# stefanopini/simple-HRNet

Hardware: AMD Instinct MI355X
Metric: person-crops/sec HRNet-W48 384x288 (model forward + heat-map decode) (higher is better)
Workload: dtype bf16; 1 GPU; HRNet-W48 384x288, batch=256 random crops per GPU, bf16 MFMA (BASELINE configs[2]); global_batch=256, micro_batch=256, lanes_per_gpu=1, parallelism=dp1 (crop sharding, RCCL all-gather of keypoints), weights=random-init seeded (synth_state_dict seed 0), BN stats randomised, engine_switches=

## Files before the change

### include/hrnet_mi355.h

```cpp
#ifndef HRNET_MI355_H
#define HRNET_MI355_H

#include <stddef.h>
#include <stdint.h>

#ifdef __cplusplus
extern "C" {
#endif

typedef struct hrn_ctx *hrn_handle;

enum { HRN_F32 = 0, HRN_BF16 = 1, HRN_F16 = 2 };
enum { HRN_BOX_I32 = 0, HRN_BOX_F32 = 1 };
enum { HRN_T_F32 = 0, HRN_T_I64 = 1 };

typedef struct {
    const char *name;
    const void *data;
    int32_t ndim;
    int64_t dims[4];
    int32_t dtype;
} hrn_tensor_desc;

typedef struct {
// ... 70 lines not shown
int hrn_preprocess_frames_yuv_dev(hrn_handle h, const hrn_yuv_frame *frames_host, int nframes, const float *dets_dev,
                                  int det_stride, const int32_t *frame_index_host, int n, int variant, float *images_dev,
                                  int32_t *boxes_dev, int32_t *status_dev, void *stream);

#define HRN_MAX_TRACKED 256
int hrn_associate_people(int P, const int32_t *cur_start, const int32_t *prev_start, int J, int32_t *boxes, float *pts,
                         const int32_t *prev_boxes, const float *prev_pts, const int32_t *prev_ids, int32_t *next_id, double pose_alpha,
                         double similarity_threshold, double smoothing_alpha, int32_t *ids, int32_t *match, int32_t *status);
const char *hrn_associate_people_last_error(void);
int hrn_associate_people_dev(hrn_handle h, int P, const int32_t *cur_start_host, const int32_t *prev_start_host, int J,
                             int32_t *boxes_dev, float *pts_dev, const int32_t *prev_boxes_dev, const float *prev_pts_dev,
                             const int32_t *prev_ids_dev, int32_t *next_id_dev, double pose_alpha, double similarity_threshold,
                             double smoothing_alpha, int32_t *ids_dev, int32_t *match_dev, int32_t *status_dev, void *stream);
int hrn_assoc_exp(const double *x, int n, double *out);
int hrn_associate_similarity(const int32_t *boxes, const float *pts, int n, const int32_t *prev_boxes, const float *prev_pts, int m, int J,
                             double pose_alpha, double *cost_out , float *sim_out );

#define HRN_POSE_NMS_SOFT 1
#define HRN_POSE_NMS_SUPPRESS 2
#define HRN_POSE_NMS_ENGINE 4
int hrn_pose_nms(int P, const int32_t *start, int J, int flags, void *kpts, void *areas, const void *scores, double thresh,
                 double in_vis_thre, double rescore_thre, const double *sigmas, int32_t *keep, int32_t *num, double *scores_out,
                 int32_t *suppressor, int32_t *status);
const char *hrn_pose_nms_last_error(void);
int hrn_pose_nms_dev(hrn_handle h, int P, const int32_t *start_host, int J, int flags, void *kpts_dev, void *areas_dev,
                     const void *scores_dev, double thresh, double in_vis_thre, double rescore_thre, const double *sigmas_dev,
                     int32_t *keep_dev, int32_t *num_dev, double *scores_out_dev, int32_t *suppressor_dev, int32_t *status_dev,
                     void *stream);
int hrn_pose_nms_oks_row(int n, int J, int flags, const void *kpts, const void *areas, int g, double in_vis_thre, const double *sigmas,
                         double *oks_out );

enum { HRN_PIX_BGR = 0 };
typedef struct { uint8_t *y, *u, *v;
                 int32_t height, width, pitch_y, pitch_c, format, matrix, range; } hrn_canvas;
int hrn_draw_poses(hrn_handle h, const hrn_canvas *canvases_host, int nframes, const float *pts_dev, int n, int J,
                   const int32_t *frame_index_host , const int32_t *skeleton_host, int K,
                   const uint8_t *point_colors_host, int Cp, const uint8_t *bone_colors_host, int Cb,
                   const int32_t *person_index_host , int radius ,
                   int thickness, float threshold, void *stream);
int hrn_draw_poses_ids_dev(hrn_handle h, const hrn_canvas *canvases_host, int nframes, const float *pts_dev, int n, int J,
                           const int32_t *frame_index_host, const int32_t *skeleton_host, int K, const uint8_t *point_colors_host,
                           int Cp, const uint8_t *bone_colors_host, int Cb, const int32_t *person_index_dev, int radius,
                           int thickness, float threshold, void *stream);
int hrn_yuv_from_bgr(int matrix, int range, const uint8_t *bgr , int n, uint8_t *yuv_out );

enum { HRN_LETTERBOX_MAX_SIDE = 0, HRN_LETTERBOX_MIN_RATIO = 1 };
enum { HRN_LB_F32 = 0, HRN_LB_F16 = 1, HRN_LB_BF16 = 2, HRN_LB_U8_HWC = 3 };
enum { HRN_LB_RGB = 0, HRN_LB_BGR = 1 };
enum { HRN_DET_COMPACT = 1 };
enum { HRN_DET_MAX_CLASSES = 16 };
typedef struct { int32_t new_w, new_h, left, top; double ratio_w, ratio_h, dw, dh; } hrn_letterbox;
int hrn_letterbox_geometry(int rule, const int32_t *frame_hw , int n, int out_h, int out_w,
                           hrn_letterbox *out );
const char *hrn_letterbox_last_error(void);
int hrn_letterbox_frames(hrn_handle h, const hrn_frame *frames_host, int n, int rule, int out_h, int out_w,
                         const uint8_t *pad , int order, int form, void *out_dev, hrn_letterbox *geometry_host ,
                         void *stream);
int hrn_letterbox_frames_yuv(hrn_handle h, const hrn_yuv_frame *frames_host, int n, int rule, int out_h, int out_w,
                             const uint8_t *pad , int order, int form, void *out_dev,
                             hrn_letterbox *geometry_host , void *stream);
int hrn_detections_to_frame(int rule, const float *dets, int det_stride, const int32_t *start , int P,
                            const hrn_letterbox *geometry, const int32_t *frame_hw , int out_h, int out_w,
                            int conf_col, float conf_thres, int class_col, const int32_t *classes, int nclasses, int flags,
                            float *dets_out, int32_t *counts_out , int32_t *status_out );
int hrn_detections_to_frame_dev(hrn_handle h, int rule, const float *dets_dev, int det_stride, const int32_t *start_host, int P,
                                const hrn_letterbox *geometry_host, const int32_t *frame_hw_host, int out_h, int out_w,
                                int conf_col, float conf_thres, int class_col, const int32_t *classes_host, int nclasses, int flags,
                                float *dets_out_dev, int32_t *counts_dev, int32_t *status_dev, void *stream);

enum { HRN_ROTATE_90_CW = 0, HRN_ROTATE_180 = 1, HRN_ROTATE_90_CCW = 2 };
int hrn_rotate_frames(hrn_handle h, const hrn_canvas *src_host, const hrn_canvas *dst_host, int nframes,
                      const int32_t *codes_host , void *stream);
int hrn_rotate_people(int n, int J, const int32_t *frame_hw , int per_person_hw,
                      const int32_t *codes , int per_person_code,
                      const float *pts , const int32_t *boxes ,
                      float *pts_out, int32_t *boxes_out);
const char *hrn_rotate_people_last_error(void);
int hrn_rotate_people_dev(hrn_handle h, int n, int J, const int32_t *frame_hw_host, int per_person_hw,
                          const int32_t *codes_host, int per_person_code, const float *pts_dev, const int32_t *boxes_dev,
                          float *pts_out_dev, int32_t *boxes_out_dev, void *stream);

enum { HRN_INTER_NEAREST = 0, HRN_INTER_LINEAR = 1, HRN_INTER_CUBIC = 2 };
int hrn_resize_frames(hrn_handle h, const uint8_t *frames_dev, int n, int frame_h, int frame_w, int interpolation,
                      float *images_dev, void *stream);

int hrn_warp_crops(hrn_handle h, const uint8_t *frames_dev, int nframes, int frame_h, int frame_w,
                   const int32_t *frame_index_host, const double *matrices_host, int n, float *images_dev, void *stream);

int hrn_forward_flip_tta(hrn_handle h, const void *images_dev, int n, const int32_t *flip_pairs_host, int npairs,
                         int post_processing, float *heatmaps_dev, float *preds_dev, float *maxvals_dev, void *stream);

int hrn_target_centers(const double *joints, const float *vis, const float *joints_weight , int n, int J,
                       int height, int width, double sigma, int32_t *mu_out, float *draw_out, float *target_weight_out);
int hrn_generate_targets(hrn_handle h, const double *joints_host, const float *vis_host, const float *joints_weight_host,
                         int n, double sigma, float *targets_dev, float *target_weight_host, void *stream);
typedef struct {
    double *loss_mse, *loss_ohkm;
    float *avg_acc;
    int32_t *cnt;
    float *acc, *dists;
    double *map_loss;
    float *preds, *target_preds, *maxvals;
} hrn_score_out;
int hrn_score_heatmaps(hrn_handle h, const float *heatmaps_dev, int n, const float *targets_dev, const double *joints_host,
                       const float *vis_host, const float *joints_weight_host, double sigma, const float *target_weight_host,
                       float pck_thr, int ohkm_topk, const hrn_score_out *out_dev, void *stream);

enum { HRN_REFINE_NONE = 0, HRN_REFINE_QUARTER = 1, HRN_REFINE_DARK = 2 };
int hrn_forward_refined(hrn_handle h, const void *images_dev, int n, const void *boxes_dev, int box_dtype, int refine,
                        float *pts_dev, float *heatmaps_dev, void *stream);
int hrn_refine_coords(hrn_handle h, const float *heatmaps_dev, int n, int refine, float *coords_dev, void *stream);

int hrn_nms(int32_t *keep_out, int32_t *num_out, const float *boxes_host, int boxes_num, int boxes_dim,
            float nms_overlap_thresh, int device_id);
int hrn_nms_release(int device_id);
const char *hrn_nms_last_error(void);

int hrn_oks_nms(int32_t *keep_out, int32_t *num_out, const double *kpts, const double *areas, const int32_t *order, int n, int J,
                double thresh, const double *sigmas, double in_vis_thre);
int hrn_soft_oks_nms(int32_t *keep_out, int32_t *num_out, const double *kpts, const double *areas, const double *scores_sorted,
                     const int32_t *order, int n, int J, double thresh, const double *sigmas, double in_vis_thre);
int hrn_pose_similarity(const double *boxes_a, const float *poses_a, int na, const double *boxes_b, const float *poses_b, int nb, int J,
                        float *sim_bbox, float *sim_pose);
int hrn_assignment(const double *cost, int rows, int cols, int32_t *row_to_col);

typedef struct {
    char name[96];
    int32_t c, h, w;
    int32_t conv_index;
} hrn_tap_info;
int hrn_tap_count(hrn_handle h);
int hrn_get_tap_info(hrn_handle h, int index, hrn_tap_info *out);
int hrn_forward_tap(hrn_handle h, const void *images_dev, int n, const char *tap_name, int crop0, int ncrops, int crop_step,
                    float *dst_dev, float *heatmaps_dev, void *stream);

int hrn_conv_count(hrn_handle h);
int hrn_get_conv_info(hrn_handle h, int index, hrn_conv_info *out);
double hrn_flops_per_crop(hrn_handle h);
int64_t hrn_workspace_bytes(hrn_handle h);
int64_t hrn_map_rebuilds(hrn_handle h);
int hrn_launches_per_pass(hrn_handle h);
int hrn_stem_fused(hrn_handle h);
int hrn_conv_compact(hrn_handle h, int index);
const char *hrn_switches(hrn_handle h);
int64_t hrn_debug_pad_violations(hrn_handle h);
int hrn_plan_block_map(hrn_handle h, int group, int n, int reverse, int32_t *blocks, int capacity, int32_t *members,
                       int member_capacity);
int hrn_plan_direct_map(hrn_handle h, int group, int n, int32_t *blocks, int capacity, int32_t *members, int member_capacity,
                        int32_t *pixels_per_tile);
int hrn_plan_s2_map(hrn_handle h, int group, int n, int32_t *blocks, int capacity, int32_t *parts, int part_capacity,
                    int32_t *active);
int hrn_plan_head_slabs(hrn_handle h, int n, int32_t *slab_px);
int hrn_plan_launch_walk(hrn_handle h, int kind, int index, int n, int32_t *out);
int hrn_profile_pass(hrn_handle h, const void *images_dev, int n, float *conv_ms, int conv_ms_len,
                     float *other_ms , void *stream);
const char *hrn_version(void);

#ifdef __cplusplus
}
#endif
#endif
```

### simple-hrnet_amd/_lib.py

```python
from __future__ import annotations

import ctypes
import os
import shutil
import subprocess
from typing import List

_HERE = os.path.dirname(os.path.abspath(__file__))
CSRC = os.path.join(_HERE, "csrc")
INCLUDE = os.path.join(os.path.dirname(_HERE), "include")
LIB_PATH = os.path.join(_HERE, "libhrnet_mi355.so")
if os.environ.get("HRN_LIB_TAG"):
    LIB_PATH = LIB_PATH.replace(".so", "_%s.so" % os.environ["HRN_LIB_TAG"])
SOURCES = ["kernels.hip", "conv3x3_lds.hip", "conv_s2.hip", "stem_fused.hip", "conv3x3_f32.hip", "bottleneck_chain.hip", "prepath.hip", "warp.hip", "nms.hip", "postproc.cpp", "hrnet_mi355.cpp",
           "decode.hip",
           "score.hip",
           "draw.hip",
           "track.hip",
           "pose_nms.hip",
           "letterbox.hip",
           "rotate.hip",
           "assoc.hip",
           "conv3x3_lds_f16.hip", "conv_s2_f16.hip", "bottleneck_chain_f16.hip"]
HEADERS = [os.path.join(CSRC, "kernels.h"), os.path.join(CSRC, "dt16.h"), os.path.join(CSRC, "argmax.h"), os.path.join(CSRC, "conv3x3_n96.inc"), os.path.join(CSRC, "conv3x3_lds.inc"),
# ... 99 lines not shown
                if verbose:
                    print(" ".join(cmd), flush=True)
                subprocess.check_call(cmd)
                with open(os.path.join(_obj_dir(), "build.stamp"), "w") as f:
                    f.write(stamp + "\n")
                os.replace(tmp, LIB_PATH)
        finally:
            fcntl.flock(lock, fcntl.LOCK_UN)
    return LIB_PATH


class TensorDesc(ctypes.Structure):
    _fields_ = [("name", ctypes.c_char_p), ("data", ctypes.c_void_p), ("ndim", ctypes.c_int32),
                ("dims", ctypes.c_int64 * 4), ("dtype", ctypes.c_int32)]


class ConvInfo(ctypes.Structure):
    _fields_ = [("name", ctypes.c_char * 96),
                ("cin", ctypes.c_int32), ("cout", ctypes.c_int32), ("ksize", ctypes.c_int32),
                ("stride", ctypes.c_int32), ("relu", ctypes.c_int32), ("has_residual", ctypes.c_int32),
                ("in_h", ctypes.c_int32), ("in_w", ctypes.c_int32), ("out_h", ctypes.c_int32),
                ("out_w", ctypes.c_int32), ("kpad", ctypes.c_int32), ("nr", ctypes.c_int32),
                ("algo", ctypes.c_int32), ("ks", ctypes.c_int32),
                ("w_offset", ctypes.c_int64), ("w_bytes", ctypes.c_int64), ("b_offset", ctypes.c_int64),
                ("flops", ctypes.c_double)]


class TapInfo(ctypes.Structure):
    _fields_ = [("name", ctypes.c_char * 96), ("c", ctypes.c_int32), ("h", ctypes.c_int32), ("w", ctypes.c_int32),
                ("conv_index", ctypes.c_int32)]


class ScoreOut(ctypes.Structure):
    _fields_ = [(name, ctypes.c_void_p) for name in ("loss_mse", "loss_ohkm", "avg_acc", "cnt", "acc", "dists", "map_loss", "preds",
                                                     "target_preds", "maxvals")]


class Frame(ctypes.Structure):
    _fields_ = [("data", ctypes.c_void_p), ("height", ctypes.c_int32), ("width", ctypes.c_int32)]


class YuvFrameC(ctypes.Structure):
    _fields_ = [("y", ctypes.c_void_p), ("u", ctypes.c_void_p), ("v", ctypes.c_void_p), ("height", ctypes.c_int32),
                ("width", ctypes.c_int32), ("pitch_y", ctypes.c_int32), ("pitch_c", ctypes.c_int32), ("format", ctypes.c_int32),
                ("matrix", ctypes.c_int32), ("range", ctypes.c_int32)]


class Letterbox(ctypes.Structure):
    _fields_ = [("new_w", ctypes.c_int32), ("new_h", ctypes.c_int32), ("left", ctypes.c_int32), ("top", ctypes.c_int32),
                ("ratio_w", ctypes.c_double), ("ratio_h", ctypes.c_double), ("dw", ctypes.c_double), ("dh", ctypes.c_double)]


class CanvasC(ctypes.Structure):
    _fields_ = list(YuvFrameC._fields_)


_P = ctypes.c_void_p
SYMBOLS = {
    "hrn_create": (ctypes.c_int, [ctypes.POINTER(_P), ctypes.c_int, ctypes.c_int, ctypes.c_int, ctypes.c_int,
                                  ctypes.c_int, ctypes.c_int, ctypes.c_int]),
    "hrn_create_model": (ctypes.c_int, [ctypes.POINTER(_P), ctypes.c_int, ctypes.c_int, ctypes.c_int, ctypes.c_int,
                                        ctypes.c_int, ctypes.c_int, ctypes.c_int, ctypes.c_int]),
    "hrn_destroy": (None, [_P]),
    "hrn_last_error": (ctypes.c_char_p, [_P]),
    "hrn_load_weights": (ctypes.c_int, [_P, ctypes.POINTER(TensorDesc), ctypes.c_int]),
    "hrn_weight_blob_bytes": (ctypes.c_int64, [_P]),
    "hrn_weight_blob_ptr": (_P, [_P]),
    "hrn_adopt_weights": (ctypes.c_int, [_P]),
    "hrn_weight_blob_read": (ctypes.c_int, [_P, ctypes.c_int64, _P, ctypes.c_int64]),
    "hrn_forward": (ctypes.c_int, [_P, _P, ctypes.c_int, _P, ctypes.c_int, _P, _P, _P]),
    "hrn_resize_frames": (ctypes.c_int, [_P, _P, ctypes.c_int, ctypes.c_int, ctypes.c_int, ctypes.c_int, _P, _P]),
    "hrn_warp_crops": (ctypes.c_int, [_P, _P, ctypes.c_int, ctypes.c_int, ctypes.c_int, _P, _P, ctypes.c_int, _P, _P]),
    "hrn_target_centers": (ctypes.c_int, [_P, _P, _P, ctypes.c_int, ctypes.c_int, ctypes.c_int, ctypes.c_int, ctypes.c_double, _P, _P, _P]),
    "hrn_generate_targets": (ctypes.c_int, [_P, _P, _P, _P, ctypes.c_int, ctypes.c_double, _P, _P, _P]),
    "hrn_score_heatmaps": (ctypes.c_int, [_P, _P, ctypes.c_int, _P, _P, _P, _P, ctypes.c_double, _P, ctypes.c_float, ctypes.c_int,
                                          ctypes.POINTER(ScoreOut), _P]),
    "hrn_preprocess_frame": (ctypes.c_int, [_P, _P, ctypes.c_int, ctypes.c_int, _P, ctypes.c_int, ctypes.c_int, ctypes.c_int, _P, _P, _P, _P]),
    "hrn_preprocess_frames": (ctypes.c_int, [_P, ctypes.POINTER(Frame), ctypes.c_int, _P, ctypes.c_int, _P, ctypes.c_int, ctypes.c_int, _P, _P, _P, _P]),
    "hrn_yuv_coefficients": (ctypes.c_int, [ctypes.c_int, ctypes.c_int, _P]),
    "hrn_yuv_to_bgr": (ctypes.c_int, [_P, ctypes.POINTER(YuvFrameC), _P, _P]),
    "hrn_preprocess_frames_yuv": (ctypes.c_int, [_P, ctypes.POINTER(YuvFrameC), ctypes.c_int, _P, ctypes.c_int, _P, ctypes.c_int, ctypes.c_int,
                                                 _P, _P, _P, _P]),
    "hrn_draw_poses": (ctypes.c_int, [_P, ctypes.POINTER(CanvasC), ctypes.c_int, _P, ctypes.c_int, ctypes.c_int, _P, _P, ctypes.c_int,
                                      _P, ctypes.c_int, _P, ctypes.c_int, _P, ctypes.c_int, ctypes.c_int, ctypes.c_float, _P]),
    "hrn_draw_poses_ids_dev": (ctypes.c_int, [_P, ctypes.POINTER(CanvasC), ctypes.c_int, _P, ctypes.c_int, ctypes.c_int, _P, _P, ctypes.c_int,
                                              _P, ctypes.c_int, _P, ctypes.c_int, _P, ctypes.c_int, ctypes.c_int, ctypes.c_float, _P]),
    "hrn_associate_people": (ctypes.c_int, [ctypes.c_int, _P, _P, ctypes.c_int, _P, _P, _P, _P, _P, _P, ctypes.c_double, ctypes.c_double,
                                            ctypes.c_double, _P, _P, _P]),
    "hrn_associate_people_last_error": (ctypes.c_char_p, []),
    "hrn_associate_people_dev": (ctypes.c_int, [_P, ctypes.c_int, _P, _P, ctypes.c_int, _P, _P, _P, _P, _P, _P, ctypes.c_double,
                                                ctypes.c_double, ctypes.c_double, _P, _P, _P, _P]),
    "hrn_assoc_exp": (ctypes.c_int, [_P, ctypes.c_int, _P]),
    "hrn_associate_similarity": (ctypes.c_int, [_P, _P, ctypes.c_int, _P, _P, ctypes.c_int, ctypes.c_int, ctypes.c_double, _P, _P]),
    "hrn_pose_nms": (ctypes.c_int, [ctypes.c_int, _P, ctypes.c_int, ctypes.c_int, _P, _P, _P, ctypes.c_double, ctypes.c_double,
                                    ctypes.c_double, _P, _P, _P, _P, _P, _P]),
    "hrn_pose_nms_last_error": (ctypes.c_char_p, []),
    "hrn_pose_nms_dev": (ctypes.c_int, [_P, ctypes.c_int, _P, ctypes.c_int, ctypes.c_int, _P, _P, _P, ctypes.c_double, ctypes.c_double,
                                        ctypes.c_double, _P, _P, _P, _P, _P, _P, _P]),
    "hrn_pose_nms_oks_row": (ctypes.c_int, [ctypes.c_int, ctypes.c_int, ctypes.c_int, _P, _P, ctypes.c_int, ctypes.c_double, _P, _P]),
    "hrn_letterbox_geometry": (ctypes.c_int, [ctypes.c_int, _P, ctypes.c_int, ctypes.c_int, ctypes.c_int, _P]),
    "hrn_letterbox_last_error": (ctypes.c_char_p, []),
    "hrn_letterbox_frames": (ctypes.c_int, [_P, ctypes.POINTER(Frame), ctypes.c_int, ctypes.c_int, ctypes.c_int, ctypes.c_int, _P, ctypes.c_int,
                                            ctypes.c_int, _P, _P, _P]),
    "hrn_letterbox_frames_yuv": (ctypes.c_int, [_P, ctypes.POINTER(YuvFrameC), ctypes.c_int, ctypes.c_int, ctypes.c_int, ctypes.c_int, _P,
                                                ctypes.c_int, ctypes.c_int, _P, _P, _P]),
    "hrn_detections_to_frame": (ctypes.c_int, [ctypes.c_int, _P, ctypes.c_int, _P, ctypes.c_int, _P, _P, ctypes.c_int, ctypes.c_int, ctypes.c_int,
                                               ctypes.c_float, ctypes.c_int, _P, ctypes.c_int, ctypes.c_int, _P, _P, _P]),
    "hrn_detections_to_frame_dev": (ctypes.c_int, [_P, ctypes.c_int, _P, ctypes.c_int, _P, ctypes.c_int, _P, _P, ctypes.c_int, ctypes.c_int,
                                                   ctypes.c_int, ctypes.c_float, ctypes.c_int, _P, ctypes.c_int, ctypes.c_int, _P, _P, _P, _P]),
    "hrn_rotate_frames": (ctypes.c_int, [_P, ctypes.POINTER(CanvasC), ctypes.POINTER(CanvasC), ctypes.c_int, _P, _P]),
    "hrn_rotate_people": (ctypes.c_int, [ctypes.c_int, ctypes.c_int, _P, ctypes.c_int, _P, ctypes.c_int, _P, _P, _P, _P]),
    "hrn_rotate_people_last_error": (ctypes.c_char_p, []),
    "hrn_rotate_people_dev": (ctypes.c_int, [_P, ctypes.c_int, ctypes.c_int, _P, ctypes.c_int, _P, ctypes.c_int, _P, _P, _P, _P, _P]),
    "hrn_yuv_from_bgr": (ctypes.c_int, [ctypes.c_int, ctypes.c_int, _P, ctypes.c_int, _P]),
    "hrn_crop_geometry": (ctypes.c_int, [_P, ctypes.c_int, ctypes.c_int, _P, ctypes.c_int, ctypes.c_int, ctypes.c_int, ctypes.c_int, _P, _P]),
    "hrn_crop_geometry_last_error": (ctypes.c_char_p, []),
    "hrn_pose_boxes": (ctypes.c_int, [_P, ctypes.c_int, ctypes.c_int, _P, ctypes.c_int, ctypes.c_float, ctypes.c_int, ctypes.c_double,
                                      ctypes.c_double, _P]),
    "hrn_pose_boxes_last_error": (ctypes.c_char_p, []),
    "hrn_boxes_from_poses": (ctypes.c_int, [_P, _P, ctypes.c_int, ctypes.c_int, _P, ctypes.c_int, ctypes.c_float, ctypes.c_int,
                                            ctypes.c_double, ctypes.c_double, _P, _P]),
    "hrn_preprocess_frames_dev": (ctypes.c_int, [_P, ctypes.POINTER(Frame), ctypes.c_int, _P, ctypes.c_int, _P, ctypes.c_int, ctypes.c_int,
                                                 _P, _P, _P, _P]),
    "hrn_preprocess_frames_yuv_dev": (ctypes.c_int, [_P, ctypes.POINTER(YuvFrameC), ctypes.c_int, _P, ctypes.c_int, _P, ctypes.c_int,
                                                     ctypes.c_int, _P, _P, _P, _P]),
    "hrn_forward_flip_tta": (ctypes.c_int, [_P, _P, ctypes.c_int, _P, ctypes.c_int, ctypes.c_int, _P, _P, _P, _P]),
    "hrn_forward_refined": (ctypes.c_int, [_P, _P, ctypes.c_int, _P, ctypes.c_int, ctypes.c_int, _P, _P, _P]),
    "hrn_refine_coords": (ctypes.c_int, [_P, _P, ctypes.c_int, ctypes.c_int, _P, _P]),
    "hrn_nms": (ctypes.c_int, [_P, _P, _P, ctypes.c_int, ctypes.c_int, ctypes.c_float, ctypes.c_int]),
    "hrn_nms_release": (ctypes.c_int, [ctypes.c_int]),
    "hrn_nms_last_error": (ctypes.c_char_p, []),
    "hrn_oks_nms": (ctypes.c_int, [_P, _P, _P, _P, _P, ctypes.c_int, ctypes.c_int, ctypes.c_double, _P, ctypes.c_double]),
    "hrn_soft_oks_nms": (ctypes.c_int, [_P, _P, _P, _P, _P, _P, ctypes.c_int, ctypes.c_int, ctypes.c_double, _P, ctypes.c_double]),
    "hrn_pose_similarity": (ctypes.c_int, [_P, _P, ctypes.c_int, _P, _P, ctypes.c_int, ctypes.c_int, _P, _P]),
    "hrn_assignment": (ctypes.c_int, [_P, ctypes.c_int, ctypes.c_int, _P]),
    "hrn_tap_count": (ctypes.c_int, [_P]),
    "hrn_get_tap_info": (ctypes.c_int, [_P, ctypes.c_int, ctypes.POINTER(TapInfo)]),
    "hrn_forward_tap": (ctypes.c_int, [_P, _P, ctypes.c_int, ctypes.c_char_p, ctypes.c_int, ctypes.c_int, ctypes.c_int, _P, _P, _P]),
    "hrn_conv_count": (ctypes.c_int, [_P]),
    "hrn_get_conv_info": (ctypes.c_int, [_P, ctypes.c_int, ctypes.POINTER(ConvInfo)]),
    "hrn_flops_per_crop": (ctypes.c_double, [_P]),
    "hrn_workspace_bytes": (ctypes.c_int64, [_P]),
    "hrn_map_rebuilds": (ctypes.c_int64, [_P]),
    "hrn_launches_per_pass": (ctypes.c_int, [_P]),
    "hrn_switches": (ctypes.c_char_p, [_P]),
    "hrn_stem_fused": (ctypes.c_int, [_P]),
    "hrn_conv_compact": (ctypes.c_int, [_P, ctypes.c_int]),
    "hrn_debug_pad_violations": (ctypes.c_int64, [_P]),
    "hrn_plan_block_map": (ctypes.c_int, [_P, ctypes.c_int, ctypes.c_int, ctypes.c_int, _P, ctypes.c_int, _P, ctypes.c_int]),
    "hrn_plan_direct_map": (ctypes.c_int, [_P, ctypes.c_int, ctypes.c_int, _P, ctypes.c_int, _P, ctypes.c_int, _P]),
    "hrn_plan_s2_map": (ctypes.c_int, [_P, ctypes.c_int, ctypes.c_int, _P, ctypes.c_int, _P, ctypes.c_int, _P]),
    "hrn_plan_head_slabs": (ctypes.c_int, [_P, ctypes.c_int, _P]),
    "hrn_plan_launch_walk": (ctypes.c_int, [_P, ctypes.c_int, ctypes.c_int, ctypes.c_int, _P]),
    "hrn_profile_pass": (ctypes.c_int, [_P, _P, ctypes.c_int, ctypes.POINTER(ctypes.c_float), ctypes.c_int,
                                        ctypes.POINTER(ctypes.c_float), _P]),
    "hrn_version": (ctypes.c_char_p, []),
}

_lib = None


def load(auto_build: bool = True) -> ctypes.CDLL:
    global _lib
    if _lib is not None:
        return _lib
    if auto_build and needs_build():
        build()
    lib = ctypes.CDLL(LIB_PATH)
    for name, (res, args) in SYMBOLS.items():
        fn = getattr(lib, name)
        fn.restype = res
        fn.argtypes = args
    _lib = lib
    return lib


def header_symbols() -> List[str]:
    import re

    text = open(os.path.join(INCLUDE, "hrnet_mi355.h")).read()
    text = re.sub(r"/\*.*?\*/", "", text, flags=re.S)
    return sorted(set(re.findall(r"\b(hrn_[a-z_0-9]+)\s*\(", text)))
```

### simple-hrnet_amd/csrc/conv3x3_lds.inc

```
typedef __attribute__((ext_vector_type(8))) __bf16 bf16x8;
typedef __attribute__((ext_vector_type(8))) short s16x8;
typedef __attribute__((ext_vector_type(4))) short s16x4;
typedef __attribute__((ext_vector_type(4))) float f32x4;
#define GLOBAL_AS __attribute__((address_space(1)))
typedef const GLOBAL_AS unsigned short *gcu16;
typedef GLOBAL_AS unsigned short *gu16;

__device__ __forceinline__ float relu1(float x) {
    float r;
    asm("v_max_f32 %0, 0, %1" : "=v"(r) : "v"(x));
    return r;
}

__device__ __forceinline__ void glds16(const GLOBAL_AS void *gsrc, char *lds_wave_base) {
    __builtin_amdgcn_global_load_lds(gsrc,
                                     (__attribute__((address_space(3))) void *)lds_wave_base, 16, 0, 0);
}

template <int KS_, int NRB_, int DT_ = DT_BF16>
struct C3Cfg {
    static constexpr int KS = KS_, NRB = NRB_;
    static constexpr int DT = DT_;
    static constexpr int PARTS = KS == 48 ? 2 : 1;
    static constexpr int CPP = KS == 48 ? 7 : 9;
// ... 299 lines not shown
                case 8: asm volatile("s_waitcnt vmcnt(8)" ::: "memory"); break;
                case 9: asm volatile("s_waitcnt vmcnt(9)" ::: "memory"); break;
                default: asm volatile("s_waitcnt vmcnt(10)" ::: "memory"); break;
            }
        }
        __builtin_amdgcn_sched_barrier(0);
        const int p0 = (mt0 + tt) * BM;
#pragma unroll
        for (int i = 0; i < MR; ++i) {
            const int q = p0 + wave * 16 * MR + i * 16 + li;
            const int n_img = (int)(((unsigned long long)(unsigned)q * p.magic_hpwp) >> p.shift_hpwp);
            const int rem = q - n_img * p.hpwp;
            const int ho = (int)(((unsigned long long)(unsigned)rem * p.magic_wp) >> p.shift_wp);
            const int wo = rem - ho * p.wp;
            const bool ok = (q < m) && (ho < p.h) && (wo < p.wd);
            const size_t o = (size_t)q * p.cout + ch0;
            unsigned pk[2 * NRB];
#pragma unroll
            for (int j = 0; j < NRB; ++j) {
                const unsigned r01 = (j >> 1) < N16 ? rpre4[i][(j >> 1) < N16 ? (j >> 1) : 0][2 * (j & 1)] : rpre2[i][0];
                const unsigned r23 = (j >> 1) < N16 ? rpre4[i][(j >> 1) < N16 ? (j >> 1) : 0][2 * (j & 1) + 1] : rpre2[i][1];
                float v0 = acc[i][j][0] + H16<DT>::lo(r01);
                float v1 = acc[i][j][1] + H16<DT>::hi(r01);
                float v2 = acc[i][j][2] + H16<DT>::lo(r23);
                float v3 = acc[i][j][3] + H16<DT>::hi(r23);
                if (p.relu) v0 = relu1(v0), v1 = relu1(v1), v2 = relu1(v2), v3 = relu1(v3);
                const unsigned lo = H16<DT>::pk(v0, v1), hi = H16<DT>::pk(v2, v3);
                pk[2 * j] = ok ? lo : 0u;
                pk[2 * j + 1] = ok ? hi : 0u;
            }
#pragma unroll
            for (int v = 0; v < N16; ++v)
                *(GLOBAL_AS u32x4 *)(out + o + v * 8) = u32x4{pk[4 * v], pk[4 * v + 1], pk[4 * v + 2], pk[4 * v + 3]};
            if (NRB & 1) *(GLOBAL_AS u32x2 *)(out + o + N16 * 8) = u32x2{pk[4 * N16], pk[4 * N16 + 1]};
        }
        after_epilogue = true;
#ifdef HRN_C3_TIMING
        C3_T(tF);
        t_epi += tF - tE;
#endif
    }
#if defined(HRN_C3_TIMING) && !defined(HRN_C3_TIMING_FUSED_ONLY)
    if (lane == 0 && g_c3_timing) {
        C3_T(t_end);
        long long *o = g_c3_timing + ((size_t)blockIdx.x * 8 + wave) * 8;
        o[0] = t_wait, o[1] = t_issue, o[2] = t_comp, o[3] = t_epi, o[4] = t_end - t_begin, o[5] = n_half, o[6] = MR,
        o[7] = S;
    }
#endif
}

constexpr int BBF_W = 14 * 3 * 1024;
constexpr int BBF_XY = 4864 * 16;
constexpr int BBF_LDS = 2 * BBF_W + BBF_XY;
static_assert(BBF_LDS <= 160 * 1024, "LDS budget");

template <int NF, int DT>
__device__ __forceinline__ void bbf_conv1(const Conv3Problem &p, const int (&xoff)[14], const int bvec, const unsigned lds0,
                                          const int row_first, const int row_last, const long q_first, const int m,
                                          const int lane, const unsigned res_a,
                                          __attribute__((ext_vector_type(2))) unsigned (&rpre)[4][3], long long &t_loop) {
    constexpr int NRB = 3, NCH = 14, ROWB = 96;
    const int li = lane & 15, g = lane >> 4;
    typedef __attribute__((ext_vector_type(2))) unsigned u32x2;
    f32x4 acc[NF][NRB];
    {
        float bias[4 * NRB];
#pragma unroll
        for (int c = 0; c < 4 * NRB; ++c) bias[c] = __int_as_float(__builtin_amdgcn_ds_bpermute((g * 4 * NRB + c) * 4, bvec));
#pragma unroll
        for (int i = 0; i < NF; ++i)
#pragma unroll
            for (int j = 0; j < NRB; ++j) acc[i][j] = f32x4{bias[j * 4], bias[j * 4 + 1], bias[j * 4 + 2], bias[j * 4 + 3]};
    }
    unsigned okbits = 0;
#pragma unroll
    for (int i = 0; i < NF; ++i) {
        const int yr = (i == NF - 1 ? row_last : row_first + i * 16) + li;
        const long q = q_first + yr;
        const unsigned uq = (unsigned)q;
        const int n_img = (int)(((unsigned long long)uq * p.magic_hpwp) >> p.shift_hpwp);
        const int rem = (int)uq - n_img * p.hpwp;
        const int ho = (int)(((unsigned long long)(unsigned)rem * p.magic_wp) >> p.shift_wp);
        const int wo = rem - ho * p.wp;
        okbits |= (q >= 0 && q < m && ho < p.h && wo < p.wd) ? 1u << i : 0u;
    }
    s16x8 wf[2][NRB], xf[2][NF];
    const unsigned wl_a = lds0 + lane * 16;
    unsigned sl_a = lds0 + 2 * BBF_W + (row_first + li) * ROWB;
    unsigned sl_z = lds0 + 2 * BBF_W + (row_last + li) * ROWB;
    asm volatile("" : "+v"(sl_a), "+v"(sl_z));
#define BBF_READ1(SET, C)                                                                                         \
    {                                                                                                             \
        _Pragma("unroll") for (int j = 0; j < NRB; ++j)                                                           \
            asm volatile("ds_read_b128 %0, %1 offset:%2" : "=v"(wf[SET][j]) : "v"(wl_a), "i"(((C)*NRB + j) * 1024)); \
        const unsigned xa = sl_a + xoff[C], xz = sl_z + xoff[C];                                                   \
        _Pragma("unroll") for (int i = 0; i < NF - 1; ++i)                                                        \
            asm volatile("ds_read_b128 %0, %1 offset:%2" : "=v"(xf[SET][i]) : "v"(xa), "i"(i * 16 * ROWB));       \
        asm volatile("ds_read_b128 %0, %1" : "=v"(xf[SET][NF - 1]) : "v"(xz));                                     \
    }
    BBF_READ1(0, 0)
#pragma unroll
    for (int c = 0; c < NCH; ++c) {
        const int cur = c & 1, nxt = cur ^ 1;
        if (c + 1 < NCH) {
            BBF_READ1(nxt, c + 1)
            asm volatile("s_waitcnt lgkmcnt(%0)" ::"i"(NRB + NF) : "memory");
        } else {
            asm volatile("s_waitcnt lgkmcnt(0)" ::: "memory");
        }
        __builtin_amdgcn_sched_barrier(0);
#pragma unroll
        for (int i = 0; i < NF; ++i)
#pragma unroll
            for (int j = 0; j < NRB; ++j)
                acc[i][j] = H16<DT>::mma(wf[cur][j], xf[cur][i], acc[i][j]);
        __builtin_amdgcn_sched_barrier(0);
    }
#undef BBF_READ1
#ifdef HRN_C3_TIMING
    t_loop = __builtin_amdgcn_s_memtime();
#endif
#pragma unroll
    for (int i = 0; i < 4; ++i)
#pragma unroll
        for (int v = 0; v < 3; ++v)
            asm volatile("ds_read_b64 %0, %1 offset:%2" : "=v"(rpre[i][v]) : "v"(res_a), "i"(i * 16 * ROWB + v * 8));
    unsigned pk[NF][2 * NRB];
#pragma unroll
    for (int i = 0; i < NF; ++i) {
        const bool ok = (okbits >> i) & 1u;
#pragma unroll
        for (int j = 0; j < NRB; ++j) {
            const unsigned lo = H16<DT>::pk(relu1(acc[i][j][0]), relu1(acc[i][j][1]));
            const unsigned hi = H16<DT>::pk(relu1(acc[i][j][2]), relu1(acc[i][j][3]));
            pk[i][2 * j] = ok ? lo : 0u;
            pk[i][2 * j + 1] = ok ? hi : 0u;
        }
    }
    asm volatile("s_waitcnt lgkmcnt(0)" ::: "memory");
    __builtin_amdgcn_s_barrier();
#pragma unroll
    for (int i = 0; i < NF; ++i) {
        const int yr = (i == NF - 1 ? row_last : row_first + i * 16) + li;
        const unsigned ya = lds0 + 2 * BBF_W + yr * ROWB + g * 24;
#pragma unroll
        for (int v = 0; v < 3; ++v)
            asm volatile("ds_write_b64 %0, %1 offset:%2" ::"v"(ya), "v"(u32x2{pk[i][2 * v], pk[i][2 * v + 1]}), "i"(v * 8) : "memory");
    }
    asm volatile("s_waitcnt lgkmcnt(0)" ::: "memory");
    __builtin_amdgcn_s_barrier();
}

template <int DT>
__device__ __forceinline__ void bbf_run(const Conv3Problem &p, const int mt0, const int tiles_this_block, const int nb, char *smem) {
    constexpr int KS = 48, NRB = 3, ROWB = 96, NCH = 14, BM = 512, MR = 4, NT = 512;
    typedef __attribute__((ext_vector_type(2))) unsigned u32x2;
    typedef __attribute__((ext_vector_type(4))) unsigned u32x4;
    const int tid = threadIdx.x, lane = tid & 63;
    const int wave = __builtin_amdgcn_readfirstlane(tid >> 6);
    const int li = lane & 15, g = lane >> 4;
    const int m = nb * p.hpwp;
    const int mtiles = (m + BM - 1) / BM;
    int ntile = mtiles - mt0;
    if (ntile > tiles_this_block) ntile = tiles_this_block;
    if (ntile <= 0) return;
    const int halo = p.wp + 1;
    const int xrows = BM + 4 * halo, yrows = BM + 2 * halo;
    const int xunits = xrows * 6;
    const int cunits = 2 * halo * 6;
    const int nfr = (yrows + 15) >> 4, base = nfr >> 3, extra = nfr & 7;
    const int cnt = base + (wave < extra ? 1 : 0);
    const int f0 = wave * base + (wave < extra ? wave : extra);
    const int row_first = f0 * 16;
    int row_last = (f0 + cnt - 1) * 16;
    if (row_last > yrows - 16) row_last = yrows - 16;
    const gcu16 in = (gcu16)p.in;
    const gu16 out = (gu16)p.out;
    const unsigned lds0 = (unsigned)(size_t)(__attribute__((address_space(3))) char *)smem;
    char *const xy = smem + 2 * BBF_W;

    int xoff[NCH];
#pragma unroll
    for (int c = 0; c < NCH; ++c) {
        int k0 = 32 * c + 8 * g;
        if (k0 >= 9 * KS) k0 = 0;
        const int tap = k0 / KS, ci = k0 - tap * KS;
        const int dh = tap / 3, dw = tap - 3 * dh;
        xoff[c] = (dh * p.wp + dw) * ROWB + (ci >> 3) * 16;
    }
    const int ch0 = g * 4 * NRB;
    const int bl = lane < KS ? lane : 0;
    const int bvec1 = __float_as_int(((const GLOBAL_AS float *)p.bias)[bl]);
    const int bvec2 = __float_as_int(((const GLOBAL_AS float *)p.bias2)[bl]);
    auto load_x = [&](int tt) {
        const long row0 = (long)(mt0 + tt) * BM - 2 * halo;
        const long lo = -(long)halo, hi = (long)m + halo + 511;
#pragma unroll
        for (int k = 0; k < BBF_XY / 16 / NT + 1; ++k) {
            if (k * NT + wave * 64 < xunits) {
                int u = k * NT + tid;
                asm volatile("" : "+v"(u));
                if (u >= xunits) u = xunits - 1;
                const int r = (int)(((unsigned)u * 43691u) >> 18);
                const int q8 = u - r * 6;
                long gr = row0 + r;
                gr = gr < lo ? lo : (gr > hi ? hi : gr);
                glds16((const GLOBAL_AS char *)(in + gr * KS + q8 * 8), xy + (k * NT + wave * 64) * 16);
            }
        }
    };
    constexpr int NXR = 6, NXP = NXR + 2;
    u32x4 xpre[NXR];
    const int xu0 = cunits;
    const int r0u = (int)(((unsigned)tid * 43691u) >> 18), q0u = tid - r0u * 6;
    auto x_src = [&](int tt, int k) {
        const int row0 = (mt0 + tt) * BM - 2 * halo;
        int r = r0u, q8 = q0u;
        asm volatile("" : "+v"(r), "+v"(q8));
        r += 2 * halo + 85 * k + (2 * k) / 6, q8 += (2 * k) % 6;
        if (q8 >= 6) q8 -= 6, ++r;
        if (r >= xrows) r = xrows - 1, q8 = 5;
        int gr = row0 + r;
        const int lo = -halo, hi = m + halo + 511;
        gr = gr < lo ? lo : (gr > hi ? hi : gr);
        return in + ((long)gr * KS + q8 * 8);
    };
    auto fetch_x = [&](int tt) {
#pragma unroll
        for (int k = 0; k < NXR; ++k) xpre[k] = *(const GLOBAL_AS u32x4 *)x_src(tt, k);
#pragma unroll
        for (int k = NXR; k < NXP; ++k)
            if (xu0 + k * NT + wave * 64 < xunits) glds16((const GLOBAL_AS char *)x_src(tt, k), xy + (xu0 + k * NT + wave * 64) * 16);
    };
    auto store_x = [&]() {
        const unsigned a0 = lds0 + 2 * BBF_W + (xu0 + tid) * 16;
        asm volatile("s_waitcnt vmcnt(0)" ::: "memory");
#pragma unroll
        for (int k = 0; k < NXR; ++k)
            asm volatile("ds_write_b128 %0, %1 offset:%2" ::"v"(a0), "v"(xpre[k]), "i"(k * NT * 16) : "memory");
    };
    u32x4 ycar[2];
    const unsigned ca0 = lds0 + 2 * BBF_W + (tid < cunits ? tid : 0) * 16;
    const unsigned ca1 = lds0 + 2 * BBF_W + (tid + NT < cunits ? tid + NT : 0) * 16;
    auto store_carry = [&]() {
        if (tid < cunits) asm volatile("ds_write_b128 %0, %1" ::"v"(ca0), "v"(ycar[0]) : "memory");
        if (tid + NT < cunits) asm volatile("ds_write_b128 %0, %1" ::"v"(ca1), "v"(ycar[1]) : "memory");
    };
    {
        const GLOBAL_AS char *w1 = (const GLOBAL_AS char *)p.w, *w2 = (const GLOBAL_AS char *)p.w2;
#pragma unroll
        for (int k = 0; k < (BBF_W / 16 + NT - 1) / NT; ++k) {
            const int u0 = k * NT + wave * 64;
            if (u0 < BBF_W / 16) {
                glds16(w1 + (size_t)(u0 + lane) * 16, smem + u0 * 16);
                glds16(w2 + (size_t)(u0 + lane) * 16, smem + BBF_W + u0 * 16);
            }
        }
        load_x(0);
    }
#ifdef HRN_C3_TIMING
    long long t_w = 0, t_c1 = 0, t_c1p = 0, t_c2 = 0, t_post = 0, t_epi = 0;
    C3_T(t_begin);
#endif
    for (int tt = 0; tt < ntile; ++tt) {
        C3_T(tA);
        if (tt == 0) asm volatile("s_waitcnt vmcnt(0)" ::: "memory");
        asm volatile("s_waitcnt lgkmcnt(0)" ::: "memory");
        __builtin_amdgcn_s_barrier();
        const long p0 = (long)(mt0 + tt) * BM;
        C3_T(tB);
        long long tC = 0;
        u32x2 rpre[MR][3];
        const unsigned res_a = lds0 + 2 * BBF_W + (wave * 16 * MR + li + 2 * halo) * ROWB + g * 24;
        const int rf = tt > 0 ? 2 * halo + wave * 64 : row_first, rl = tt > 0 ? rf + 48 : row_last;
        if (tt == 0 && cnt == 6)
            bbf_conv1<6, DT>(p, xoff, bvec1, lds0, rf, rl, p0 - halo, m, lane, res_a, rpre, tC);
        else if (tt == 0 && cnt == 5)
            bbf_conv1<5, DT>(p, xoff, bvec1, lds0, rf, rl, p0 - halo, m, lane, res_a, rpre, tC);
        else
            bbf_conv1<4, DT>(p, xoff, bvec1, lds0, rf, rl, p0 - halo, m, lane, res_a, rpre, tC);
        C3_T(tD);
        const bool carry = tt + 1 < ntile;
        if (carry) fetch_x(tt + 1);
        unsigned okbits2 = 0;
#pragma unroll
        for (int i = 0; i < MR; ++i) {
            const int q = (int)p0 + wave * 16 * MR + i * 16 + li;
            const int n_img = (int)(((unsigned long long)(unsigned)q * p.magic_hpwp) >> p.shift_hpwp);
            const int rem = q - n_img * p.hpwp;
            const int ho = (int)(((unsigned long long)(unsigned)rem * p.magic_wp) >> p.shift_wp);
            const int wo = rem - ho * p.wp;
            okbits2 |= ((q < m) && (ho < p.h) && (wo < p.wd)) ? 1u << i : 0u;
        }
        __builtin_amdgcn_sched_barrier(0);
        f32x4 acc[MR][NRB];
        {
            float bias2[4 * NRB];
#pragma unroll
            for (int c = 0; c < 4 * NRB; ++c) bias2[c] = __int_as_float(__builtin_amdgcn_ds_bpermute((ch0 + c) * 4, bvec2));
#pragma unroll
            for (int i = 0; i < MR; ++i)
#pragma unroll
                for (int j = 0; j < NRB; ++j) acc[i][j] = f32x4{bias2[j * 4], bias2[j * 4 + 1], bias2[j * 4 + 2], bias2[j * 4 + 3]};
        }
        {
            s16x8 wf[2][NRB], xf[2][MR];
            const unsigned wl_a = lds0 + BBF_W + lane * 16;
            unsigned sl_a = lds0 + 2 * BBF_W + (wave * 16 * MR + li) * ROWB;
            asm volatile("" : "+v"(sl_a));
#define BBF_READ2(SET, C)                                                                                         \
    {                                                                                                             \
        _Pragma("unroll") for (int j = 0; j < NRB; ++j)                                                           \
            asm volatile("ds_read_b128 %0, %1 offset:%2" : "=v"(wf[SET][j]) : "v"(wl_a), "i"(((C)*NRB + j) * 1024)); \
        const unsigned xa = sl_a + xoff[C];                                                                        \
        _Pragma("unroll") for (int i = 0; i < MR; ++i)                                                            \
            asm volatile("ds_read_b128 %0, %1 offset:%2" : "=v"(xf[SET][i]) : "v"(xa), "i"(i * 16 * ROWB));       \
    }
            BBF_READ2(0, 0)
#pragma unroll
            for (int c = 0; c < NCH; ++c) {
                const int cur = c & 1, nxt = cur ^ 1;
                if (c + 1 < NCH) {
                    BBF_READ2(nxt, c + 1)
                    asm volatile("s_waitcnt lgkmcnt(%0)" ::"i"(NRB + MR) : "memory");
                } else {
                    asm volatile("s_waitcnt lgkmcnt(0)" ::: "memory");
                    if (carry) {
                        asm volatile("ds_read_b128 %0, %1 offset:%2" : "=v"(ycar[0]) : "v"(ca0), "i"(BM * ROWB) : "memory");
                        asm volatile("ds_read_b128 %0, %1 offset:%2" : "=v"(ycar[1]) : "v"(ca1), "i"(BM * ROWB) : "memory");
                    }
                }
                __builtin_amdgcn_sched_barrier(0);
#pragma unroll
                for (int i = 0; i < MR; ++i)
#pragma unroll
                    for (int j = 0; j < NRB; ++j)
                        acc[i][j] = H16<DT>::mma(wf[cur][j], xf[cur][i], acc[i][j]);
                __builtin_amdgcn_sched_barrier(0);
            }
#undef BBF_READ2
        }
        C3_T(tE);
        asm volatile("s_waitcnt lgkmcnt(0)" ::: "memory");
        __builtin_amdgcn_s_barrier();
        if (carry) {
            store_carry();
            store_x();
        }
        __builtin_amdgcn_sched_barrier(0);
        C3_T(tF);
#pragma unroll
        for (int i = 0; i < MR; ++i) {
            const int q = (int)p0 + wave * 16 * MR + i * 16 + li;
            const bool ok = (okbits2 >> i) & 1u;
            const size_t o = (size_t)q * KS + ch0;
            unsigned pk[2 * NRB];
#pragma unroll
            for (int j = 0; j < NRB; ++j) {
                const unsigned r01 = rpre[i][j][0], r23 = rpre[i][j][1];
                float v0 = acc[i][j][0] + H16<DT>::lo(r01);
                float v1 = acc[i][j][1] + H16<DT>::hi(r01);
                float v2 = acc[i][j][2] + H16<DT>::lo(r23);
                float v3 = acc[i][j][3] + H16<DT>::hi(r23);
                if (p.relu) v0 = relu1(v0), v1 = relu1(v1), v2 = relu1(v2), v3 = relu1(v3);
                const unsigned lo = H16<DT>::pk(v0, v1), hi = H16<DT>::pk(v2, v3);
                pk[2 * j] = ok ? lo : 0u;
                pk[2 * j + 1] = ok ? hi : 0u;
            }
            *(GLOBAL_AS u32x4 *)(out + o) = u32x4{pk[0], pk[1], pk[2], pk[3]};
            *(GLOBAL_AS u32x2 *)(out + o + 8) = u32x2{pk[4], pk[5]};
        }
#ifdef HRN_C3_TIMING
        C3_T(tG);
        t_w += tB - tA, t_c1 += tC - tB, t_c1p += tD - tC, t_c2 += tE - tD, t_post += tF - tE, t_epi += tG - tF;
#endif
    }
#ifdef HRN_C3_TIMING
    if (lane == 0 && g_c3_timing) {
        C3_T(t_end);
        long long *o = g_c3_timing + ((size_t)blockIdx.x * 8 + wave) * 8;
        o[0] = t_w, o[1] = t_c1, o[2] = t_c1p, o[3] = t_c2, o[4] = t_end - t_begin, o[5] = ntile, o[6] = 100 + cnt,
        o[7] = t_post | (t_epi << 32);
    }
#endif
}

#include "conv3x3_n96.inc"

template <int KS, int NRB, int DT>
__global__ __launch_bounds__(512, 2) void conv3x3_lds_kernel(const Conv3Problem *__restrict__ probs,
                                                             const int2 *__restrict__ blockmap, const int nb) {
    extern __shared__ __attribute__((aligned(16))) char smem[];
    using CFG = C3Cfg<KS, NRB, DT>;
#ifdef HRN_Q_TIMING
    struct Stamp {
        long long t0;
        __device__ Stamp() : t0((long long)__builtin_amdgcn_s_memrealtime()) {}
        __device__ ~Stamp() {
            if (g_q_timing && threadIdx.x == 0) {
                unsigned hw, xcc;
                asm volatile("s_getreg_b32 %0, hwreg(HW_REG_HW_ID)\n\ts_getreg_b32 %1, hwreg(HW_REG_XCC_ID)" : "=s"(hw), "=s"(xcc));
                const int seq = g_q_seq;
                long long *o = g_q_timing + ((size_t)(seq & (kQSlots - 1)) * kQBlocks + (blockIdx.x < kQBlocks ? blockIdx.x : kQBlocks - 1)) * 4;
                o[0] = t0, o[1] = (long long)gridDim.x | ((long long)seq << 32), o[2] = (long long)__builtin_amdgcn_s_memrealtime();
                o[3] = (long long)(((xcc & 15u) << 16) | (hw & 0xff00u));
            }
        }
    } stamp_;
#endif
    const int2 bm = blockmap[blockIdx.x];
    const Conv3Problem p = probs[bm.x & 0xff];
    const int nt = (bm.x >> 8) & 0xff, tiles = bm.x >> 16;
    const int mt0 = bm.y & 0x1fffffff;
    if constexpr (KS == 48 && NRB == 3) {
        if (bm.y & (1 << 29)) {
            bbf_run<DT>(p, mt0, tiles, nb, smem);
            return;
        }
        if (p.n96) {
            if (p.compact) {
                if (bm.y >> 30)
                    c3n_run<1, true, DT>(p, nt, mt0, tiles, nb, smem);
                else
                    c3n_run<4, true, DT>(p, nt, mt0, tiles, nb, smem);
                return;
            }
            if (bm.y >> 30)
                c3n_run<1, false, DT>(p, nt, mt0, tiles, nb, smem);
            else if (p.bm == 512)
                c3n_run<4, false, DT>(p, nt, mt0, tiles, nb, smem);
            else
                c3n_run<3, false, DT>(p, nt, mt0, tiles, nb, smem);
            return;
        }
    }
    if (bm.y >> 30) {
        conv3_run<CFG, 1>(p, nt, mt0, tiles, nb, smem);
    } else if constexpr (NRB == 4) {
        conv3_run<CFG, 3>(p, nt, mt0, tiles, nb, smem);
    } else {
        if (p.bm == 512)
            conv3_run<CFG, 4>(p, nt, mt0, tiles, nb, smem);
        else
            conv3_run<CFG, 3>(p, nt, mt0, tiles, nb, smem);
    }
}

template <int KS, int NRB, int DT>
static hipError_t launch_c3(const Conv3Problem *probs_dev, const int2 *blockmap_dev, int nblocks, int nb, hipStream_t s) {
    using CFG = C3Cfg<KS, NRB, DT>;
    constexpr int LDS = (KS == 48 && NRB == 3) ? (BBF_LDS > N96_LDS ? BBF_LDS : N96_LDS) : CFG::LDS;
    static_assert(LDS >= CFG::LDS, "LDS budget");
    static std::atomic<unsigned long long> lds_set{0};
    {
        const hipError_t e = set_dynamic_lds((const void *)conv3x3_lds_kernel<KS, NRB, DT>, LDS, lds_set);
        if (e != hipSuccess) return e;
    }
#ifdef HRN_Q_TIMING
    hipLaunchKernelGGL(q_seq_bump, dim3(1), dim3(1), 0, s);
#endif
    hipLaunchKernelGGL((conv3x3_lds_kernel<KS, NRB, DT>), dim3(nblocks), dim3(512), LDS, s, probs_dev, blockmap_dev, nb);
    return hipGetLastError();
}

template <int DT>
static hipError_t launch_conv3x3_lds_t(const Conv3Problem *probs_dev, const void *blockmap_dev, int nblocks, int nb, int ks, int nrb,
                                       hipStream_t s) {
    if (nblocks <= 0) return hipSuccess;
    const int2 *bm = (const int2 *)blockmap_dev;
    if ((ks == 48 && nrb == 3) || (ks == 32 && nrb == 6)) return launch_c3<48, 3, DT>(probs_dev, bm, nblocks, nb, s);
    if (ks == 32 && nrb == 4) return launch_c3<32, 4, DT>(probs_dev, bm, nblocks, nb, s);
    if (ks == 32 && nrb == 3) return launch_c3<32, 3, DT>(probs_dev, bm, nblocks, nb, s);
    if (ks == 32 && nrb == 2) return launch_c3<32, 2, DT>(probs_dev, bm, nblocks, nb, s);
    return hipErrorInvalidValue;
}
```

### simple-hrnet_amd/csrc/ctx_memory.inc

```
    bool hip_ok(hipError_t e, const char *what) {
        if (e == hipSuccess) return true;
        err = std::string(what) + ": " + hipGetErrorString(e);
        return false;
    }
    bool refuse_plan_only() {
        if (plan_only) err = "plan-only handle (device_id < 0): there is no CPU compute path";
        return plan_only;
    }

    bool allocate() {
        workspace_bytes = 0;
        for (auto &b : buffers) workspace_bytes += (int64_t)b.bytes;
        const int64_t small_crops = std::min<int64_t>(max_batch, (191 + head_slabs) / head_slabs);
        const int64_t part = std::max((int64_t)max_batch * joints * head_slabs, small_crops * joints * head_slabs_small);
        workspace_bytes += part * 8;
        if (plan_only) {
            fill_problems();
            index_s2groups();
            blob = (char *)mmap(nullptr, (size_t)blob_bytes, PROT_READ | PROT_WRITE, MAP_PRIVATE | MAP_ANONYMOUS, -1, 0);
            if (blob == (char *)MAP_FAILED) blob = nullptr;
            return blob != nullptr;
        }
        if (!hip_ok(hipSetDevice(device), "hipSetDevice")) return false;
        for (auto &b : buffers) {
            if (!hip_ok(hipMalloc((void **)&b.dev, b.bytes), "hipMalloc(activation)")) return false;
            if (!hip_ok(hipMemset(b.dev, 0, b.bytes), "hipMemset(activation)")) return false;
        }
        if (!hip_ok(hipMalloc((void **)&blob, (size_t)blob_bytes), "hipMalloc(weights)")) return false;
        if (!hip_ok(hipMemset(blob, 0, (size_t)blob_bytes), "hipMemset(weights)")) return false;
        if (!setup_groups() || !setup_dgroups() || !setup_s2groups()) return false;
        if (!hip_ok(hipMalloc((void **)&part_val, (size_t)part * 4), "hipMalloc(part_val)")) return false;
        if (!hip_ok(hipMalloc((void **)&part_idx, (size_t)part * 4), "hipMalloc(part_idx)")) return false;
        return hip_ok(hipDeviceSynchronize(), "hipDeviceSynchronize");
    }

    int conv3_tiles_per_block(const ConvOp &cv) const {
        if (cv.n96) return std::max(1, (half_stages_per_block * 7) / (6 * 3 * cv.slices));
        const int t = half_stages_per_block / ((cv.ks == 48 ? 2 : 1) * cv.slices);
        return t < 1 ? 1 : t;
    }

    bool bbf_active(const ConvOp &cv, int nb) const {
        return (nb * tensors[cv.out_t].hpwp + 511) / 512 >= bbf_min_tiles;
    }
    bool fused_now(const ConvOp &cv, int nb) const { return cv.fuse_with >= 0 && bbf_active(cv, nb); }
    bool skipped(const ConvOp &cv, int nb) const { return cv.fused_away && bbf_active(cv, nb); }

    int group_blocks(const Conv3Group &g, int nb, std::vector<int2> *out, bool reverse, bool all_short = false,
                     std::vector<int> *tile_px_out = nullptr) const {
        struct Ent {
            double key;
            int2 v;
            int bm;
        };
        std::vector<Ent> ents;
        long one_per_block = 0;
        for (int ci : g.conv_idx) {
            const ConvOp &cv = convs[ci];
            if (skipped(cv, nb)) continue;
            const Tensor &to = tensors[cv.out_t];
            const int bmn = fused_now(cv, nb) ? 512 : conv3x3_lds_bm(cv.ks, cv.nr, to.wp);
            one_per_block += (long)((m_pixels(cv, to, nb) + bmn - 1) / bmn) * cv.ntiles;
        }
        const bool small = small_tiles && one_per_block < small_below;
        long small_blocks = 0;
        for (int ci : g.conv_idx) {
            const ConvOp &cv = convs[ci];
            if (skipped(cv, nb)) continue;
            small_blocks += (long)((m_pixels(cv, tensors[cv.out_t], nb) + 127) / 128) * cv.ntiles;
        }
        const bool keep_short_full = small && small_keep_above > 0 && small_blocks > small_keep_above;
        auto short_conv = [&](const ConvOp &cv) { return cv.ks != 16 && !cv.n96 && (cv.ks == 48 ? 2 : 1) * cv.slices <= 2; };
        auto small_conv = [&](const ConvOp &cv) {
            if (cv.ks == 16 && f32_small_slices > 0 && cv.slices >= f32_small_slices) return true;
            return small && !(keep_short_full && short_conv(cv));
        };
        auto tile_px = [&](const ConvOp &cv, const Tensor &to) {
            return fused_now(cv, nb) ? 512 : small_conv(cv) ? 128 : conv3x3_lds_bm(cv.ks, cv.nr, to.wp);
        };
        auto tiles_per_block = [&](const ConvOp &cv, int div) {
            return std::max(1, conv3_tiles_per_block(cv) / (fused_now(cv, nb) ? bbf_tpb_div : 1) / div);
        };
        auto count_blocks = [&](int div) {
            long total = 0;
            for (int ci : g.conv_idx) {
                const ConvOp &cv = convs[ci];
                if (skipped(cv, nb)) continue;
                const Tensor &to = tensors[cv.out_t];
                const int bm = tile_px(cv, to);
                const int mtiles = (int)((m_pixels(cv, to, nb) + bm - 1) / bm);
                const int tpb = tiles_per_block(cv, div);
                total += (long)((mtiles + tpb - 1) / tpb) * cv.ntiles;
            }
            return total;
        };
        int div = 1;
        while (div < 64 && count_blocks(div) < 512) div *= 2;
        int lf = all_short ? 1 : (int)std::min<long>(long_factor, count_blocks(div) / 768);
        if (lf < 1) lf = 1;
        for (size_t k = 0; k < g.conv_idx.size(); ++k) {
            const ConvOp &cv = convs[g.conv_idx[k]];
            if (skipped(cv, nb)) continue;
            const Tensor &to = tensors[cv.out_t];
            const int bm = tile_px(cv, to);
            const bool fused = fused_now(cv, nb);
            const int prob = fused ? g.fused_prob[k] : (int)k;
            const int mtiles = (int)((m_pixels(cv, to, nb) + bm - 1) / bm);
            const int tpb_short = tiles_per_block(cv, div);
            const int tpb_long = tpb_short * lf;
            const int long_tiles = ((int)(mtiles * long_share) / (8 * tpb_long)) * (8 * tpb_long);
            for (int phase = 0; phase < 2; ++phase) {
                const int tpb = phase == 0 ? tpb_long : tpb_short;
                const int first = phase == 0 ? 0 : long_tiles;
                const int count = phase == 0 ? long_tiles : mtiles - long_tiles;
                if (count <= 0) continue;
                const int mgroups = (count + tpb - 1) / tpb;
                const int total = mgroups * cv.ntiles;
                int seq = 0;
                for (int round = 0; round * 8 < mgroups; ++round)
                    for (int nt = 0; nt < cv.ntiles; ++nt)
                        for (int x = 0; x < 8; ++x) {
                            const int mg = round * 8 + x;
                            if (mg >= mgroups) continue;
                            const int i = seq++;
                            int tiles = count - mg * tpb;
                            if (tiles > tpb) tiles = tpb;
                            double key = (i + 0.5) / total;
                            if (block_order == 1)
                                key = -(fused ? 28000.0 + (tiles - 1) * bbf_slide_cost
                                        : (double)tiles * (cv.ks == 16 ? cv.slices * (double)bm * 36.0 + 2000.0
                                                        : cv.n96      ? cv.slices * 3.0 * (bm == 512 ? 3900.0 : 3000.0) + (bm == 512 ? 7000.0 : 5000.0)
                                                                 : cv.slices * 2.0 * (bm == 512 ? 4300.0 : 3500.0) + (bm == 512 ? 5000.0 : 3000.0))) +
                                      1e-3 * key;
                            int mt0 = first + mg * tpb;
                            if (reverse) mt0 = mtiles - mt0 - tiles;
                            ents.push_back({key, int2{prob | (nt << 8) | (tiles << 16), mt0 | (fused ? 1 << 29 : small_conv(cv) ? 1 << 30 : 0)}, bm});
                        }
            }
        }
        std::stable_sort(ents.begin(), ents.end(), [](const Ent &a, const Ent &b) { return a.key < b.key; });
        if (tile_px_out) {
            tile_px_out->resize(ents.size());
            for (size_t i = 0; i < ents.size(); ++i) (*tile_px_out)[i] = ents[i].bm;
        }
        if (out) {
            out->resize(ents.size());
            for (size_t i = 0; i < ents.size(); ++i) (*out)[i] = ents[i].v;
        }
        return (int)ents.size();
    }

    const Tensor &grid_of(const ConvOp &cv) const { return tensors[cv.up ? cv.in_t : cv.out_t]; }

    ConvArgs conv_args(const ConvOp &cv, int nb, bool rev) const {
        const Tensor &ti = tensors[cv.in_t], &to = grid_of(cv);
        ConvArgs a;
        a.in = row0(cv.in_t), a.out = row0(cv.out_t);
        a.w = blob + cv.w_off, a.bias = (const float *)(blob + cv.b_off);
        a.res = cv.res_t >= 0 ? row0(cv.res_t) : nullptr;
        a.cin = cv.cin, a.cout = cv.cout;
        a.in_wp = ti.wp, a.in_hpwp = ti.hpwp;
        a.out_h = to.h, a.out_w = to.w, a.out_wp = to.wp, a.out_hpwp = to.hpwp;
        a.m = nb * to.hpwp;
        a.ksize = cv.k, a.stride = cv.stride, a.relu = cv.relu, a.kchunks = cv.kchunks;
        a.rev = rev;
        a.pre_mode = pre_mode;
        a.wlds = direct_wlds && is16() ? 1 : 0;
        a.xlds = conv_xl(cv) ? 1 : 0;
        a.up = cv.up ? 1 : 0, a.up_a = cv.up ? (cv.up - 1) >> 1 : 0, a.up_b = cv.up ? (cv.up - 1) & 1 : 0;
        a.up_wp = tensors[cv.out_t].wp, a.up_hpwp = tensors[cv.out_t].hpwp;
        for (int t = 0; t < 4; ++t) {
            const int dy = (t >> 1) - 1 + a.up_a, dx = (t & 1) - 1 + a.up_b;
            a.taps[t] = cv.up ? dy * ti.wp + dx : 0;
        }
        return a;
    }

    int direct_group_blocks(const DirectGroup &g, int nb, std::vector<int2> *out, int mr = 4) const {
        struct Cls {
            int in_t, k, stride;
            std::vector<int> members;
            double cost = 0;
        };
        std::vector<Cls> cls;
        for (size_t k = 0; k < g.conv_idx.size(); ++k) {
            const ConvOp &cv = convs[g.conv_idx[k]];
            size_t ci = 0;
            for (; ci < cls.size(); ++ci)
                if (cls[ci].in_t == cv.in_t && cls[ci].k == cv.k && cls[ci].stride == cv.stride) break;
            if (ci == cls.size()) cls.push_back(Cls{cv.in_t, cv.k, cv.stride, {}, 0});
            cls[ci].members.push_back((int)k);
            cls[ci].cost += (double)grid_of(cv).hpwp * (cv.cout / (16 * g.nr)) * cv.kchunks;
        }
        std::stable_sort(cls.begin(), cls.end(), [](const Cls &a, const Cls &b) { return a.cost > b.cost; });
        int n = 0;
        if (out) out->clear();
        for (const Cls &cl : cls) {
            const int mtiles = (nb * grid_of(convs[g.conv_idx[cl.members[0]]]).hpwp + 64 * mr - 1) / (64 * mr);
            for (int round = 0; round * 8 < mtiles; ++round)
                for (int k : cl.members) {
                    const int ngroups = convs[g.conv_idx[k]].cout / (16 * g.nr);
                    for (int ng = 0; ng < ngroups; ++ng)
                        for (int x = 0; x < 8; ++x, ++n)
                            if (out) out->push_back(int2{k | (ng << 8), round * 8 + x});
                }
        }
        return n;
    }

    int64_t m_pixels(const ConvOp &cv, const Tensor &to, int nb) const {
        return cv.compact ? (int64_t)nb * to.h * to.w : (int64_t)nb * to.hpwp;
    }
    static int compact_slab_rows(int h, int w, int bm, int crops) {
        const int wp = w + 1, hpwp = (h + 1) * wp, hw = h * w;
        auto flat = [&](int64_t c) { const int64_t n = c / hw, r = c % hw; return n * hpwp + (r / w) * wp + r % w; };
        const int64_t m = (int64_t)crops * hw;
        int64_t span = 0;
        for (int64_t c0 = 0; c0 < m; c0 += bm) span = std::max(span, flat(std::min(c0 + bm, m) - 1) - flat(c0) + 1);
        return (int)span + 2 * wp + 2;
    }

    bool setup_dgroups() {
        for (auto &g : dgroups) {
            g.map_capacity = std::max<int64_t>(direct_group_blocks(g, max_batch, nullptr), 4 * 512 + 64 * (int64_t)g.conv_idx.size() * 8);
            for (MapSlot &sl : g.slot) {
                if (!alloc_slot(sl, g.map_capacity, g.conv_idx.size())) return false;
                workspace_bytes += g.map_capacity * (int64_t)sizeof(int2) + (int64_t)(g.conv_idx.size() * sizeof(ConvArgs));
            }
        }
        return true;
    }

    size_t index_s2groups() {
        size_t n = 0;
        for (auto &g : s2groups) g.prob_first = (int)n, n += g.probs.size();
        if (stem_fuse) stemf.prob_first = (int)n, n += stemf.probs.size();
        return n;
    }
    long s2_tiles(const S2Group &g, int nb) const {
        long t = 0;
        for (auto &pr : g.probs) t += (long)nb * pr.tiles_per_image;
        return t;
    }
    bool s2_active(const S2Group &g, int nb) const { return s2_tiles(g, nb) >= s2_min_tiles; }
    int s2_blocks(const S2Group &g, int nb, std::vector<int2> *out) const {
        struct Ent {
            double key;
            int2 v;
        };
        std::vector<double> cost(g.probs.size());
        double total = 0;
        for (size_t k = 0; k < g.probs.size(); ++k) {
            const S2Group::Prob &pr = g.probs[k];
            const Tensor &to = tensors[convs[pr.parts[0].first].out_t];
            const int frags = (pr.rows * to.wp + 15) / 16;
// ... 30 lines not shown
        std::vector<W> ws;
        for (int p = 0; p < nparts; ++p) {
            const int m = std::max(1, 8 / nparts + (p < 8 % nparts ? 1 : 0));
            for (int i = 0; i < m && (int)ws.size() < 8; ++i) ws.push_back({p, i, m});
        }
        std::stable_sort(ws.begin(), ws.end(), [](const W &a, const W &b) { return a.m < b.m; });
        double load[4] = {0, 0, 0, 0};
        bool used[8] = {};
        for (int w = 0; w < 8; ++w) part[w] = 0xff, f0[w] = 0, fs[w] = 1;
        for (const W &x : ws) {
            int best = -1;
            for (int w = 0; w < 8; ++w)
                if (!used[w] && (best < 0 || load[w & 3] < load[best & 3] - 1e-12)) best = w;
            used[best] = true;
            load[best & 3] += 1.0 / x.m;
            part[best] = (unsigned char)x.p, f0[best] = (unsigned char)x.i, fs[best] = (unsigned char)x.m;
        }
    }

    bool setup_s2groups() {
        const size_t nprob = index_s2groups();
        if (!nprob) return true;
        std::vector<S2Problem> hp(nprob);
        std::vector<S2Group *> all;
        for (auto &g : s2groups) all.push_back(&g);
        if (stem_fuse) all.push_back(&stemf);
        for (S2Group *gp : all) {
            S2Group &g = *gp;
            for (size_t k = 0; k < g.probs.size(); ++k) {
                const S2Group::Prob &pr = g.probs[k];
                const Tensor &ti = tensors[pr.in_t], &to = tensors[convs[pr.parts[0].first].out_t];
                S2Problem &q = hp[g.prob_first + k];
                memset(&q, 0, sizeof q);
                q.in = row0(pr.in_t), q.cin = ti.c, q.in_wp = ti.wp, q.in_hpwp = ti.hpwp;
                q.ho = to.h, q.wo = to.w, q.wop = to.wp, q.out_hpwp = to.hpwp;
                q.rows = pr.rows, q.tiles_per_image = pr.tiles_per_image;
                q.nparts = (int)pr.parts.size();
                s2_wave_table(q.nparts, q.wave_part, q.wave_f0, q.wave_fs);
                if (gp == &stemf)
                    for (int w = 0; w < 8; ++w)
                        if (q.wave_part[w] == 1 && q.wave_fs[w] == 4) q.wave_f0[w] = (unsigned char)((q.wave_f0[w] + 2) & 3);
                fast_div(to.wp, &q.magic_wop, &q.shift_wop);
                for (int i = 0; i < q.nparts; ++i) {
                    const ConvOp &cv = convs[pr.parts[i].first];
                    S2Part &pt = q.part[i];
                    const int nf = s2_frags_per_part(cv.cin);
                    pt.w = blob + cv.w2_off + (int64_t)pr.parts[i].second * ((9 * cv.cin + 31) / 32) * nf * 1024;
                    pt.bias = (const float *)(blob + cv.b_off);
                    pt.out = row0(cv.out_t);
                    pt.cout = cv.cout, pt.ch0 = pr.parts[i].second * 16 * nf, pt.relu = cv.relu;
                }
            }
            g.map_capacity = 64;
            for (auto &pr : g.probs) g.map_capacity += (int64_t)max_batch * pr.tiles_per_image;
            for (MapSlot &sl : g.slot) {
                if (!alloc_slot(sl, g.map_capacity, 0)) return false;
                workspace_bytes += g.map_capacity * (int64_t)sizeof(int2);
            }
        }
        if (!hip_ok(hipMalloc((void **)&s2probs_dev, nprob * sizeof(S2Problem)), "hipMalloc(s2 problems)")) return false;
        return hip_ok(hipMemcpy(s2probs_dev, hp.data(), nprob * sizeof(S2Problem), hipMemcpyHostToDevice), "hipMemcpy(s2 problems)");
    }

    bool alloc_slot(MapSlot &sl, int64_t capacity, size_t nargs) {
        if (!hip_ok(hipMalloc((void **)&sl.dev, (size_t)capacity * sizeof(int2)), "hipMalloc(blockmap)")) return false;
        if (!hip_ok(hipHostMalloc((void **)&sl.pin, (size_t)capacity * sizeof(int2), hipHostMallocDefault), "hipHostMalloc(blockmap)"))
            return false;
        if (nargs) {
            if (!hip_ok(hipMalloc((void **)&sl.args_dev, nargs * sizeof(ConvArgs)), "hipMalloc(conv args)")) return false;
            if (!hip_ok(hipHostMalloc((void **)&sl.args_pin, nargs * sizeof(ConvArgs), hipHostMallocDefault), "hipHostMalloc(conv args)"))
                return false;
        }
        return hip_ok(hipEventCreateWithFlags(&sl.landed, hipEventDisableTiming), "hipEventCreate");
    }
    void free_slot(MapSlot &sl) {
        if (sl.dev) (void)hipFree(sl.dev);
        if (sl.pin) (void)hipHostFree(sl.pin);
        if (sl.args_dev) (void)hipFree(sl.args_dev);
        if (sl.args_pin) (void)hipHostFree(sl.args_pin);
        if (sl.landed) (void)hipEventDestroy(sl.landed);
        sl = MapSlot();
    }
    MapSlot *find_slot(MapSlot (&slots)[kMapSlots], int nb, bool *hit) {
        MapSlot *lru = &slots[0];
        for (MapSlot &sl : slots) {
            if (sl.nb == nb) {
                sl.stamp = ++map_clock;
                *hit = true;
                return &sl;
            }
            if (sl.stamp < lru->stamp) lru = &sl;
        }
        *hit = false;
        if (lru->nb >= 0) (void)hipEventSynchronize(lru->landed);
        lru->nb = -1;
        lru->stamp = ++map_clock;
        return lru;
    }

    hipError_t slot_ready(MapSlot *sl, bool hit, hipStream_t s) {
        if (hit && sl->up_stream != s) return hipStreamWaitEvent(s, sl->landed, 0);
        if (!hit) sl->up_stream = s;
        return hipSuccess;
    }

    size_t index_groups() {
        size_t nprob = 0;
        for (auto &g : groups) {
            g.prob_first = (int)nprob;
            nprob += g.conv_idx.size();
            g.fused_prob.assign(g.conv_idx.size(), -1);
            int extra = (int)g.conv_idx.size();
            for (size_t k = 0; k < g.conv_idx.size(); ++k)
                if (convs[g.conv_idx[k]].fuse_with >= 0) g.fused_prob[k] = extra++, ++nprob;
        }
        return nprob;
    }

    size_t fill_problems() {
        const size_t nprob = index_groups();
        probs_host.assign(nprob, Conv3Problem{});
        std::vector<Conv3Problem> &hp = probs_host;
        for (auto &g : groups) {
            g.max_wp = 0;
            for (size_t k = 0; k < g.conv_idx.size(); ++k) {
                const ConvOp &cv = convs[g.conv_idx[k]];
                const Tensor &to = tensors[cv.out_t];
                Conv3Problem &q = hp[g.prob_first + k];
                q.in = row0(cv.in_t), q.out = row0(cv.out_t);
                q.w = blob + cv.w_off, q.bias = (const float *)(blob + cv.b_off);
                q.res = cv.res_t >= 0 ? row0(cv.res_t) : nullptr;
                q.cin = cv.cin, q.cout = cv.cout, q.h = to.h, q.wd = to.w, q.wp = to.wp, q.hpwp = to.hpwp;
                q.relu = cv.relu, q.slices = cv.slices, q.ntiles = cv.ntiles;
                q.w2 = nullptr, q.bias2 = nullptr;
                q.n96 = cv.n96 ? 1 : 0;
                q.compact = cv.compact ? 1 : 0, q.hw = to.h * to.w;
                q.slab_rows = q.slab_rows_small = 0;
                if (cv.compact) {
                    fast_div(q.hw, &q.magic_hw, &q.shift_hw);
                    fast_div(to.w, &q.magic_w, &q.shift_w);
                    q.slab_rows = compact_slab_rows(to.h, to.w, 512, max_batch), q.slab_rows_small = compact_slab_rows(to.h, to.w, 128, max_batch);
                }
                q.tiles_per_block = conv3_tiles_per_block(cv);
                q.bm = conv3x3_lds_bm(cv.ks, cv.nr, to.wp);
                fast_div(to.hpwp, &q.magic_hpwp, &q.shift_hpwp);
                fast_div(to.wp, &q.magic_wp, &q.shift_wp);
                if (to.wp > g.max_wp) g.max_wp = to.wp;
                if (cv.fuse_with >= 0) {
                    const ConvOp &c2 = convs[cv.fuse_with];
                    Conv3Problem &f = hp[g.prob_first + g.fused_prob[k]];
                    f = q;
                    f.out = row0(c2.out_t), f.relu = c2.relu, f.res = nullptr;
                    f.w2 = blob + c2.w_off, f.bias2 = (const float *)(blob + c2.b_off);
                }
            }
        }
        return nprob;
    }

    bool setup_groups() {
        const size_t nprob = fill_problems();
        if (!nprob) return true;
        std::vector<Conv3Problem> &hp = probs_host;
        for (auto &g : groups) {
            g.map_capacity = 64 + 4 * (int64_t)std::max(small_below, 256) + 1024;
            for (int ci : g.conv_idx) {
                const ConvOp &cv = convs[ci];
                const Tensor &to = tensors[cv.out_t];
                const int bm = f32_small_slices > 0 ? 128 : conv3x3_lds_bm(cv.ks, cv.nr, to.wp);
                g.map_capacity += (int64_t)((max_batch * to.hpwp + bm - 1) / bm) * cv.ntiles;
            }
            for (MapSlot &sl : g.slot) {
                if (!alloc_slot(sl, g.map_capacity, 0)) return false;
                workspace_bytes += g.map_capacity * (int64_t)sizeof(int2);
            }
        }
        if (!hip_ok(hipMalloc((void **)&probs_dev, nprob * sizeof(Conv3Problem)), "hipMalloc(problems)")) return false;
        return hip_ok(hipMemcpy(probs_dev, hp.data(), nprob * sizeof(Conv3Problem), hipMemcpyHostToDevice),
                      "hipMemcpy(problems)");
    }

    void free_all() {
        if (plan_only) {
            if (blob) (void)munmap(blob, (size_t)blob_bytes);
        } else {
            (void)hipSetDevice(device);
            for (auto &b : buffers)
                if (b.dev) (void)hipFree(b.dev);
            if (blob) (void)hipFree(blob);
            if (scratch_hm) (void)hipFree(scratch_hm);
            free_scratch();
            if (part_val) (void)hipFree(part_val);
            if (part_idx) (void)hipFree(part_idx);
            if (probs_dev) (void)hipFree(probs_dev);
            if (s2probs_dev) (void)hipFree(s2probs_dev);
            for (auto &g : s2groups)
                for (MapSlot &sl : g.slot) free_slot(sl);
            for (MapSlot &sl : stemf.slot) free_slot(sl);
            for (auto &g : groups)
                for (MapSlot &sl : g.slot) free_slot(sl);
            for (auto &g : dgroups)
                for (MapSlot &sl : g.slot) free_slot(sl);
        }
        blob = nullptr;
    }

    char *row0(int t) const {
        const Tensor &tt = tensors[t];
        const Buffer &b = buffers[tt.buf];
        return b.dev ? b.dev + b.lead_rows * tt.c * esize : nullptr;
    }
```

### simple-hrnet_amd/csrc/ctx_plan.inc

```
    int new_tensor(int ch, int h, int w) {
        Tensor t;
        t.c = ch, t.h = h, t.w = w, t.wp = w + 1, t.hp = h + 1, t.hpwp = t.wp * t.hp;
        for (size_t i = 0; i < buffers.size(); ++i)
            if (!buffers[i].in_use && buffers[i].c == ch && buffers[i].h == h && buffers[i].w == w) {
                t.buf = (int)i;
                break;
            }
        if (t.buf < 0) {
            Buffer b;
            b.c = ch, b.h = h, b.w = w;
            b.lead_rows = (size_t)t.wp + 1;
            b.rows = b.lead_rows + (size_t)max_batch * t.hpwp + t.wp + 1 + kConvBlockRows;
            b.bytes = (size_t)align_up((int64_t)(b.rows * ch * esize), 256);
            buffers.push_back(b);
            t.buf = (int)buffers.size() - 1;
        }
        buffers[t.buf].in_use = true;
        tensors.push_back(t);
        return (int)tensors.size() - 1;
    }
    void release(int t) { buffers[tensors[t].buf].in_use = false; }

    int default_nr(int cout, int stride) const {
        int nr = (cout % 64 == 0) ? 4 : (cout % 48 == 0) ? 3 : 2;
        if (is16() && stride == 2 && cout % 96 == 0 && direct_nr6) nr = 6;
        return nr;
    }
    int common_nr(const std::vector<int> &couts, int stride) const {
        bool all64 = true, all48 = true, all96 = true;
        for (int co : couts) all64 &= co % 64 == 0, all48 &= co % 48 == 0, all96 &= co % 96 == 0;
        if (is16() && stride == 2 && all96 && direct_nr6) return 6;
        return all64 ? 4 : all48 ? 3 : 2;
    }

    static int s2_rows(int wop, int ho, int cin) {
        const int r = (s2_slot_capacity(cin) - 2 * wop) / s2_pair_pitch(wop);
        return r > ho ? ho : (r < 0 ? 0 : r);
    }

    int add_conv(const std::string &conv, const std::string &bn, int in_t, int cout, int k, int stride, int relu,
                 int res_t = -1, bool emit = true, int nr_override = 0, int up = 0, int up_out_t = -1, bool force_generic = false) {
        const Tensor ti = tensors[in_t];
        ConvOp op;
        op.conv = conv, op.bn = bn, op.in_t = in_t, op.res_t = res_t;
        op.cin = ti.c, op.cout = cout, op.k = k, op.stride = stride, op.relu = relu;
        const int oh = ti.h / stride, ow = ti.w / stride;
        op.up = up;
        op.out_t = up ? up_out_t : new_tensor(cout, oh, ow);
        const int kc = is16() ? 32 : 16;
        const int K = k * k * op.cin;
        op.kchunks = (K + kc - 1) / kc;
        op.kpad = op.kchunks * kc;
        op.nr = nr_override ? nr_override : default_nr(cout, stride);
        op.flops = 2.0 * cout * (double)K * oh * ow;
        int lds_ks = 0, lds_nrb = 0;
        if (is16() && k == 3 && stride == 1 && !disable_lds && !up && !force_generic) {
            const int64_t out_bytes = ((int64_t)max_batch * (oh + 1) * (ow + 1) + 2 * (ow + 2) + 512) * std::max(op.cin, cout) * 2;
            if (!disable_n96 && op.cin % 32 == 0 && cout % 96 == 0 && conv3x3_lds_bm(32, 6, ow + 1) > 0 && out_bytes < (int64_t(1) << 32))
                lds_ks = 32, lds_nrb = 6, op.n96 = true;
            else if (op.cin % 48 == 0 && cout % 48 == 0)
                lds_ks = 48, lds_nrb = 3;
            else if (op.cin % 32 == 0 && !disable_lds32)
                lds_ks = 32, lds_nrb = cout % 64 == 0 ? 4 : cout % 48 == 0 ? 3 : cout % 32 == 0 ? 2 : 0;
            if (lds_nrb && conv3x3_lds_bm(lds_ks, lds_nrb, ow + 1) == 0) lds_nrb = 0;
            if (op.n96 && lds_nrb == 6 && !disable_compact && conv3x3_lds_bm(32, 6, ow + 1) == 512 &&
                1.0 - (double)(oh * ow) / ((oh + 1) * (ow + 1)) >= compact_min_pad &&
                (compact_slab_rows(oh, ow, 512, max_batch) + 15) / 16 * 16 <= conv3x3_n96_max_rows() && (int64_t)max_batch * oh * ow < (int64_t(1) << 27))
                op.compact = true;
        }
        if (lds_nrb) {
            op.algo = 1, op.ks = lds_ks, op.nr = lds_nrb;
            op.slices = op.cin / lds_ks, op.ntiles = cout / (16 * lds_nrb), op.nch = (9 * lds_ks + 31) / 32;
            op.kpad = op.nch * 32 * op.slices;
        }
        if (dtype == HRN_F32 && k == 3 && stride == 1 && !up && !disable_lds && !disable_f32lds && op.cin % 16 == 0 &&
            (cout % 48 == 0 || cout % 32 == 0) && conv3x3_lds_bm(16, cout % 48 == 0 ? 3 : 2, ow + 1) > 0) {
            op.algo = 1, op.ks = 16, op.nr = cout % 48 == 0 ? 3 : 2;
            op.slices = op.cin / 16, op.ntiles = cout / (16 * op.nr), op.nch = 9;
            op.kpad = 9 * 16 * op.slices;
        }
        if (is16() && k == 3 && stride == 2 && (op.cin == 48 || op.cin == 32 || op.cin == 64) &&
            cout % (16 * s2_frags_per_part(op.cin)) == 0 && !up && !disable_s2 && op.algo == 0 &&
            (s2_rows(ow + 1, oh, op.cin) >= 2 || s2_rows(ow + 1, oh, op.cin) == oh))
            op.s2 = true;
        convs.push_back(op);
        if (emit) emit_convs({(int)convs.size() - 1});
        return op.out_t;
    }

    static int c3_family(const ConvOp &cv) { return ((cv.ks == 48 && cv.nr == 3) || cv.n96) ? 0 : cv.ks * 16 + cv.nr; }

    void emit_direct(const std::vector<int> &idx, std::vector<Op> &dst) {
        std::vector<std::vector<int>> dsets;
        for (int i : idx) {
            if (disable_dgroup) {
                dst.push_back({OP_CONV, i});
                continue;
            }
            bool placed = false;
            for (auto &set : dsets)
                if (convs[set[0]].nr == convs[i].nr && set.size() < 255) {
                    set.push_back(i);
                    placed = true;
                    break;
                }
            if (!placed) dsets.push_back({i});
        }
        for (auto &set : dsets) {
            if (set.size() == 1) {
                dst.push_back({OP_CONV, set[0]});
                continue;
            }
            DirectGroup g;
            g.conv_idx = set, g.nr = convs[set[0]].nr;
            dgroups.push_back(g);
            dst.push_back({OP_CONV_GROUP, (int)dgroups.size() - 1});
        }
    }

    void emit_convs(const std::vector<int> &idx) {
        std::vector<int> lds, direct, s2;
        for (int i : idx) {
            if (convs[i].algo == 1)
                lds.push_back(i);
            else if (convs[i].s2)
                s2.push_back(i);
            else
                direct.push_back(i);
        }
        emit_direct(direct, ops);
        if (!s2.empty()) {
            S2Group g;
            g.conv_idx = s2;
            for (int i : s2) {
                const ConvOp &cv = convs[i];
                for (int t = 0; t < cv.cout / (16 * s2_frags_per_part(cv.cin)); ++t) {
                    S2Group::Prob *pr = nullptr;
                    for (auto &q : g.probs)
                        if (q.in_t == cv.in_t && (int)q.parts.size() < kS2MaxParts) pr = &q;
                    if (!pr) {
                        g.probs.push_back(S2Group::Prob());
                        pr = &g.probs.back();
                        pr->in_t = cv.in_t;
                        const Tensor &to = tensors[cv.out_t];
                        pr->rows = s2_rows(to.wp, to.h, cv.cin);
                        pr->tiles_per_image = (to.h + pr->rows - 1) / pr->rows;
                    }
                    pr->parts.push_back({i, t});
                }
            }
            emit_direct(s2, g.fallback);
            s2groups.push_back(g);
            ops.push_back({OP_S2_GROUP, (int)s2groups.size() - 1});
        }
        if (lds.empty()) return;
        std::vector<std::vector<int>> sets;
        for (int i : lds) {
            bool placed = false;
            if (!disable_group)
                for (auto &set : sets)
                    if (c3_family(convs[set[0]]) == c3_family(convs[i])) {
                        set.push_back(i);
                        placed = true;
                        break;
                    }
            if (!placed) sets.push_back({i});
        }
        for (auto &set : sets) {
            Conv3Group g;
            g.conv_idx = set;
            groups.push_back(g);
            ops.push_back({OP_CONV3_GROUP, (int)groups.size() - 1});
        }
    }

    int add_fuse(const std::vector<int> &terms, const std::vector<int> &shifts, const std::string &name) {
        FuseOp f;
        f.name = name;
        f.nterms = (int)terms.size();
        for (int i = 0; i < f.nterms; ++i) f.term_t[i] = terms[i], f.shift[i] = shifts[i];
        const Tensor &t0 = tensors[terms[0]];
        int ref = -1;
        for (int i = 0; i < f.nterms; ++i)
            if (shifts[i] == 0) ref = terms[i];
        const Tensor &tr = tensors[ref >= 0 ? ref : terms[0]];
        (void)t0;
        f.out_t = new_tensor(tr.c, tr.h, tr.w);
        fuses.push_back(f);
        return f.out_t;
    }

    void add_stage(const std::string &name, std::vector<int> &xs, int nout) {
        const int nb = (int)xs.size();
        char buf[160];
        for (int k = 0; k < 4; ++k) {
            std::vector<int> t1(nb), g1, g2;
            for (int b = 0; b < nb; ++b) {
                snprintf(buf, sizeof buf, "%s.branches.%d.%d", name.c_str(), b, k);
                const std::string p = buf;
                t1[b] = add_conv(p + ".conv1", p + ".bn1", xs[b], c << b, 3, 1, 1, -1, false);
                g1.push_back((int)convs.size() - 1);
            }
            emit_convs(g1);
            for (int b = 0; b < nb; ++b) {
                snprintf(buf, sizeof buf, "%s.branches.%d.%d", name.c_str(), b, k);
                const std::string p = buf;
                const int t2 = add_conv(p + ".conv2", p + ".bn2", t1[b], c << b, 3, 1, 1, xs[b], false);
                const int i2 = (int)convs.size() - 1, i1 = g1[b];
                const ConvOp &a1 = convs[i1], &a2 = convs[i2];
                if (!disable_bbf && is16() && a1.algo == 1 && a2.algo == 1 && a1.ks == 48 && a1.nr == 3 && a1.slices == 1 &&
                    a1.ntiles == 1 && a2.slices == 1 && a2.ntiles == 1 && conv3x3_lds_bbf_ok(tensors[t2].wp)) {
                    convs[i1].fuse_with = i2;
                    convs[i2].fused_away = true;
                }
                g2.push_back(i2);
                release(t1[b]);
                release(xs[b]);
                xs[b] = t2;
            }
            emit_convs(g2);
        }
        std::vector<std::vector<int>> term(nout, std::vector<int>(nb, -1));
        std::vector<std::vector<int>> cur(nout, std::vector<int>(nb, -1));
        for (int level = 0; level < nb; ++level) {
            std::vector<int> made, dead;
            for (int j = 0; j < nb; ++j) {
                std::vector<int> c1, c2;
                if (level == 0)
                    for (int i = 0; i < nout && i < j; ++i) c1.push_back(c << i);
                for (int i = j + 1 + level; i < nout; ++i)
                    if (level == 0) c2.push_back(i - j == 1 ? (c << i) : (c << j));
                const int nr1 = (dgroup_nr_mode == 1 && c1.size() > 1) ? common_nr(c1, 1) : 0;
                const int nr2 = (dgroup_nr_mode == 1 && c2.size() > 1) ? common_nr(c2, 2) : 0;
                for (int i = 0; i < nout; ++i) {
                    snprintf(buf, sizeof buf, "%s.fuse_layers.%d.%d", name.c_str(), i, j);
                    const std::string q = buf;
                    if (i < j && level == 0) {
                        term[i][j] = add_conv(q + ".0", q + ".1", xs[j], c << i, 1, 1, 0, -1, false, nr1);
                        made.push_back((int)convs.size() - 1);
                    } else if (i > j && level < i - j) {
                        const bool last = (level == i - j - 1);
                        snprintf(buf, sizeof buf, "%s.%d", q.c_str(), level);
                        const std::string qq = buf;
                        const int src = level == 0 ? xs[j] : cur[i][j];
                        const int nt = add_conv(qq + ".0", qq + ".1", src, last ? (c << i) : (c << j), 3, 2, last ? 0 : 1, -1,
                                                false, level == 0 ? nr2 : 0);
                        made.push_back((int)convs.size() - 1);
                        if (level > 0) dead.push_back(src);
                        cur[i][j] = nt;
                        if (last) term[i][j] = nt;
                    }
                }
            }
            if (made.empty()) break;
            emit_convs(made);
            for (int t : dead) release(t);
        }
        std::vector<int> outs;
        for (int i = 0; i < nout; ++i) {
            std::vector<int> terms, shifts;
            for (int j = 0; j < nb; ++j) {
                terms.push_back(i == j ? xs[j] : term[i][j]);
                shifts.push_back(i < j ? j - i : 0);
            }
            snprintf(buf, sizeof buf, "%s.fuse.%d", name.c_str(), i);
            outs.push_back(add_fuse(terms, shifts, buf));
        }
        {
            const int first = (int)fuses.size() - nout;
            for (int i = 0; i < nout; ++i) {
                fuses[first + i].group = disable_fgroup ? 1 : (i == 0 ? nout : 0);
                if (fuses[first + i].group) ops.push_back({OP_FUSE, first + i});
            }
        }
        for (int i = 0; i < nout; ++i)
            for (int j = 0; j < nb; ++j)
                if (i != j) release(term[i][j]);
        for (int b = 0; b < nb; ++b) release(xs[b]);
        xs = outs;
    }

    int add_layer1(int x, int nblocks) {
        char buf[96];
        int o1_next = -1;
        for (int b = 0; b < nblocks; ++b) {
            snprintf(buf, sizeof buf, "layer1.%d", b);
            const std::string p = buf;
            int o1 = o1_next, r = x;
            const bool chain = is16() && !disable_chain && b < nblocks - 1;
            int ds_idx = -1;
            if (b == 0 && chain && !disable_chain_ds) {
                o1 = add_conv(p + ".conv1", p + ".bn1", x, 64, 1, 1, 1);
                r = add_conv(p + ".downsample.0", p + ".downsample.1", x, 256, 1, 1, 0, -1, false, 2);
                ds_idx = (int)convs.size() - 1;
                release(r);
            } else if (b == 0) {
                o1 = add_conv(p + ".conv1", p + ".bn1", x, 64, 1, 1, 1, -1, false);
                r = add_conv(p + ".downsample.0", p + ".downsample.1", x, 256, 1, 1, 0, -1, false);
                emit_convs({(int)convs.size() - 2, (int)convs.size() - 1});
            } else if (o1 < 0) {
                o1 = add_conv(p + ".conv1", p + ".bn1", x, 64, 1, 1, 1);
            }
            const bool c2_generic = is16() && b >= 1;
            const bool chain3 = c2_generic && !disable_chain && !disable_chain3;
            const int o2 = c2_generic ? add_conv(p + ".conv2", p + ".bn2", o1, 64, 3, 1, 1, -1, !chain3, 2, 0, -1, true)
                                      : add_conv(p + ".conv2", p + ".bn2", o1, 64, 3, 1, 1);
            const int i2 = (int)convs.size() - 1;
            int o3;
            o1_next = -1;
            if (chain3 && !chain) {
                o3 = add_conv(p + ".conv3", p + ".bn3", o2, 256, 1, 1, 1, r, false, 2);
                chains.push_back({(int)convs.size() - 1, -1, -1, i2});
                ops.push_back({OP_CHAIN, (int)chains.size() - 1});
            } else if (chain) {
                snprintf(buf, sizeof buf, "layer1.%d", b + 1);
                const std::string pn = buf;
                o3 = add_conv(p + ".conv3", p + ".bn3", o2, 256, 1, 1, 1, r, false, 2);
                const int i3 = (int)convs.size() - 1;
                o1_next = add_conv(pn + ".conv1", pn + ".bn1", o3, 64, 1, 1, 1, -1, false, 4);
                chains.push_back({i3, (int)convs.size() - 1, ds_idx, chain3 ? i2 : -1});
                ops.push_back({OP_CHAIN, (int)chains.size() - 1});
            } else {
                o3 = add_conv(p + ".conv3", p + ".bn3", o2, 256, 1, 1, 1, r);
            }
            release(o1), release(o2);
            if (b == 0 && ds_idx < 0) release(r);
            release(x);
            x = o3;
        }
        return x;
    }

    void build_plan_poseresnet() {
        static const int spec50[4] = {3, 4, 6, 3}, spec101[4] = {3, 4, 23, 3}, spec152[4] = {3, 8, 36, 3};
        const int *layers = c == 50 ? spec50 : c == 101 ? spec101 : spec152;
        stem_out_t = new_tensor(64, H / 2, W / 2);
        ops.push_back({OP_STEM7, 0});
        int x = new_tensor(64, H / 4, W / 4);
        pool_in_t = stem_out_t, pool_out_t = x;
        ops.push_back({OP_MAXPOOL, 0});
        release(stem_out_t);
        char buf[96];
        x = add_layer1(x, layers[0]);
        for (int li = 1; li < 4; ++li) {
            const int planes = 64 << li;
            for (int b = 0; b < layers[li]; ++b) {
                snprintf(buf, sizeof buf, "layer%d.%d", li + 1, b);
                const std::string p = buf;
                const int stride = (b == 0 && li > 0) ? 2 : 1;
                int r = x;
                const int o1 = add_conv(p + ".conv1", p + ".bn1", x, planes, 1, 1, 1, -1, false);
                std::vector<int> first{(int)convs.size() - 1};
                if (b == 0) {
                    r = add_conv(p + ".downsample.0", p + ".downsample.1", x, planes * 4, 1, stride, 0, -1, false);
                    first.push_back((int)convs.size() - 1);
                }
                emit_convs(first);
                const int o2 = add_conv(p + ".conv2", p + ".bn2", o1, planes, 3, stride, 1);
                const int o3 = add_conv(p + ".conv3", p + ".bn3", o2, planes * 4, 1, 1, 1, r);
                release(o1), release(o2);
                if (b == 0) release(r);
                release(x);
                x = o3;
            }
        }
        for (int i = 0; i < 3; ++i) {
            const Tensor tx = tensors[x];
            const int up_t = new_tensor(256, tx.h * 2, tx.w * 2);
            snprintf(buf, sizeof buf, "deconv_layers.%d", 3 * i);
            const std::string cn = buf;
            snprintf(buf, sizeof buf, "deconv_layers.%d", 3 * i + 1);
            const std::string bn = buf;
            std::vector<int> phases;
            for (int ph = 0; ph < 4; ++ph) {
                add_conv(cn, bn, x, 256, 2, 1, 1, -1, false, 0, 1 + ph, up_t);
                phases.push_back((int)convs.size() - 1);
            }
            emit_convs(phases);
            release(x);
            x = up_t;
        }
        head_in_t = x;
        head_c = tensors[x].c;
        ops.push_back({OP_HEAD, 0});
        ops.push_back({OP_DECODE, 0});
        layout_blob();
    }

    void build_plan() {
        if (model == 1) return build_plan_poseresnet();
        head_c = c;
        stem_out_t = new_tensor(64, H / 2, W / 2);
        ops.push_back({OP_STEM, 0});
        int x = add_conv("conv2", "bn2", stem_out_t, 64, 3, 2, 1);
        stem_conv2_op = (int)ops.size() - 1;
        if (is16() && !disable_stem_fuse && !disable_stem_mfma && stem_fused_fits(tensors[x].wp, W)) {
            stem_fuse = true;
            convs.back().w2_image = true;
            stemf = S2Group();
            stemf.conv_idx = {(int)convs.size() - 1};
            for (int t = 0; t < 2; ++t) {
                if (stemf.probs.empty()) {
                    stemf.probs.push_back(S2Group::Prob());
                    stemf.probs[0].in_t = stem_out_t;
                    stemf.probs[0].rows = 1, stemf.probs[0].tiles_per_image = tensors[x].h;
                }
                stemf.probs[0].parts.push_back({(int)convs.size() - 1, t});
            }
        }
        release(stem_out_t);
        char buf[96];
        x = add_layer1(x, 4);
        std::vector<int> xs;
        xs.push_back(add_conv("transition1.0.0", "transition1.0.1", x, c, 3, 1, 1, -1, false));
        xs.push_back(add_conv("transition1.1.0.0", "transition1.1.0.1", x, 2 * c, 3, 2, 1, -1, false));
        emit_convs({(int)convs.size() - 2, (int)convs.size() - 1});
        release(x);
        add_stage("stage2.0", xs, 2);
        xs.push_back(add_conv("transition2.2.0.0", "transition2.2.0.1", xs[1], 4 * c, 3, 2, 1));
        for (int m = 0; m < 4; ++m) {
            snprintf(buf, sizeof buf, "stage3.%d", m);
            add_stage(buf, xs, 3);
        }
        xs.push_back(add_conv("transition3.3.0.0", "transition3.3.0.1", xs[2], 8 * c, 3, 2, 1));
        add_stage("stage4.0", xs, 4);
        add_stage("stage4.1", xs, 4);
        add_stage("stage4.2", xs, 1);
        head_in_t = xs[0];
        ops.push_back({OP_HEAD, 0});
        ops.push_back({OP_DECODE, 0});

        layout_blob();
    }

    void index_taps() {
        taps.clear();
        auto add = [&](const std::string &name, int tensor, int op, int conv) {
            for (TapPoint &t : taps)
                if (t.name == name) {
                    t.op = op;
                    return;
                }
            taps.push_back(TapPoint{name, tensor, op, conv});
        };
        for (size_t oi = 0; oi < ops.size(); ++oi) {
            const Op &op = ops[oi];
            switch (op.kind) {
                case OP_STEM:
                case OP_STEM7: add("stem", stem_out_t, (int)oi, -1); break;
                case OP_MAXPOOL: add("maxpool", pool_out_t, (int)oi, -1); break;
                case OP_CONV: add(convs[op.idx].conv, convs[op.idx].out_t, (int)oi, op.idx); break;
                case OP_CONV3_GROUP:
                    for (int ci : groups[op.idx].conv_idx) add(convs[ci].conv, convs[ci].out_t, (int)oi, ci);
                    break;
                case OP_CONV_GROUP:
                    for (int ci : dgroups[op.idx].conv_idx) add(convs[ci].conv, convs[ci].out_t, (int)oi, ci);
                    break;
                case OP_S2_GROUP:
                    for (int ci : s2groups[op.idx].conv_idx) add(convs[ci].conv, convs[ci].out_t, (int)oi, ci);
                    break;
                case OP_CHAIN:
                    add(convs[chains[op.idx].conv3].conv, convs[chains[op.idx].conv3].out_t, (int)oi, chains[op.idx].conv3);
                    if (chains[op.idx].conv1 >= 0)
                        add(convs[chains[op.idx].conv1].conv, convs[chains[op.idx].conv1].out_t, (int)oi, chains[op.idx].conv1);
                    break;
                case OP_FUSE:
                    for (int k = 0; k < fuses[op.idx].group; ++k) add(fuses[op.idx + k].name, fuses[op.idx + k].out_t, (int)oi, -1);
                    break;
                default: break;
            }
        }
    }

    void layout_blob() {
        int64_t off = 0;
        stem_w_off = off, off = align_up(off + (model == 1 ? 147 : 27) * 64 * 4, 256);
        stem_b_off = off, off = align_up(off + 64 * 4, 256);
        stem_wp_off = off, off = align_up(off + (model == 1 ? 5 : 1) * 4 * 1024, 256);
        for (auto &cv : convs) {
            cv.w_off = off;
            cv.w_bytes = cv.algo == 1 ? (int64_t)cv.ntiles * cv.slices * cv.nch * cv.nr * 1024
                                      : (int64_t)(cv.cout / 16) * cv.kchunks * 1024;
            off = align_up(off + cv.w_bytes, 256);
            cv.b_off = off;
            off = align_up(off + cv.cout * 4, 256);
            if (cv.s2 || cv.w2_image) {
                const int nf = s2_frags_per_part(cv.cin);
                cv.w2_off = off;
                cv.w2_bytes = (int64_t)(cv.cout / (16 * nf)) * ((9 * cv.cin + 31) / 32) * nf * 1024;
                off = align_up(off + cv.w2_bytes, 256);
            }
        }
        head_w_off = off, off = align_up(off + (int64_t)joints * head_c * 4, 256);
        head_b_off = off, off = align_up(off + joints * 4, 256);
        head_wp_off = off, off = align_up(off + (int64_t)((joints + 31) / 32) * 2 * ((head_c + 31) / 32) * 1024, 256);
        blob_bytes = off;

        const int hw = (H / 4) * (W / 4);
        head_slab_px = 1024;
        head_slabs = (hw + head_slab_px - 1) / head_slab_px;
        head_slabs_small = (hw + kHeadSlabPxSmall - 1) / kHeadSlabPxSmall;
    }
```

### simple-hrnet_amd/csrc/ctx_run.inc

```
    struct Timing {
        std::vector<hipEvent_t> ev;
    };

    bool run_pass(const float *images, int nb, const void *boxes, int box_dtype, float *pts, float *heatmaps,
                  hipStream_t s, Timing *tm, int flip = 0, const TapReq *tap = nullptr, int refine = RF_NONE) {
        if (tm && !hip_ok(hipEventRecord(tm->ev[0], s), "hipEventRecord")) return false;
        const bool fused_stem = stem_fuse && !(tap && tap->op == 0);
        for (size_t oi = 0; oi < ops.size(); ++oi) {
            const bool rev = alternate && (oi & 1);
            hipError_t e = hipSuccess;
            if (fused_stem && oi == 0)
                e = exec_stem_fused(images, nb, s, flip);
            else if (!(fused_stem && (int)oi == stem_conv2_op))
                e = exec_op(ops[oi], rev, images, nb, boxes, box_dtype, pts, heatmaps, s, flip, refine);
            if (!hip_ok(e, "kernel launch")) return false;
            if (tap && tap->op == (int)oi) {
                const Tensor &t = tensors[tap->tensor];
                TapArgs a;
                a.in = row0(tap->tensor), a.dst = tap->dst;
                a.c = t.c, a.h = t.h, a.w = t.w, a.wp = t.wp, a.hpwp = t.hpwp;
                a.crop0 = tap->crop0, a.ncrops = tap->ncrops, a.crop_step = tap->crop_step;
                if (!hip_ok(launch_tap(dtype, a, s), "tap launch")) return false;
            }
            if (tm && !hip_ok(hipEventRecord(tm->ev[oi + 1], s), "hipEventRecord")) return false;
        }
        return true;
    }

    hipError_t exec_stem_fused(const float *images, int nb, hipStream_t s, int flip) {
        S2Group &g = stemf;
        bool hit;
        MapSlot *sl = find_slot(g.slot, nb, &hit);
        hipError_t e = slot_ready(sl, hit, s);
        if (e != hipSuccess) return e;
        if (!hit) {
            sl->nblocks = s2_blocks(g, nb, &g.map_host);
            if (sl->nblocks > g.map_capacity) return hipErrorInvalidValue;
            memcpy(sl->pin, g.map_host.data(), (size_t)sl->nblocks * sizeof(int2));
            e = hipMemcpyAsync(sl->dev, sl->pin, (size_t)sl->nblocks * sizeof(int2), hipMemcpyHostToDevice, s);
            if (e == hipSuccess) e = hipEventRecord(sl->landed, s);
            if (e != hipSuccess) return e;
            sl->nb = nb;
            ++map_builds;
        }
        const Tensor &t = tensors[stem_out_t];
        StemArgs a;
        a.images = images, a.out = nullptr;
        a.w = nullptr, a.bias = (const float *)(blob + stem_b_off), a.wp = (const void *)(blob + stem_wp_off);
        a.n = nb, a.H = H, a.W = W;
        a.out_h = t.h, a.out_w = t.w, a.out_wp = t.wp, a.out_hpwp = t.hpwp;
        a.flip = flip;
        return launch_stem_fused(dtype, s2probs_dev + g.prob_first, sl->dev, sl->nblocks, a, s);
    }

    hipError_t exec_op(const Op &op, bool rev, const float *images, int nb, const void *boxes, int box_dtype, float *pts,
                       float *heatmaps, hipStream_t s, int flip, int refine) {
        hipError_t e = hipSuccess;
        switch (op.kind) {
        case OP_STEM: {
            const Tensor &t = tensors[stem_out_t];
            StemArgs a;
            a.images = images, a.out = row0(stem_out_t);
            a.w = (const float *)(blob + stem_w_off), a.bias = (const float *)(blob + stem_b_off);
            a.wp = (is16() && !disable_stem_mfma) ? (const void *)(blob + stem_wp_off) : nullptr;
            a.n = nb, a.H = H, a.W = W;
            a.out_h = t.h, a.out_w = t.w, a.out_wp = t.wp, a.out_hpwp = t.hpwp;
            a.flip = flip;
            e = launch_stem(dtype, a, s);
            break;
        }
        case OP_STEM7: {
            const Tensor &t = tensors[stem_out_t];
            Stem7Args a;
            a.images = images, a.out = row0(stem_out_t);
            a.w = (const float *)(blob + stem_w_off), a.bias = (const float *)(blob + stem_b_off);
            a.wp = (is16() && !disable_stem_mfma) ? (const void *)(blob + stem_wp_off) : nullptr;
            a.n = nb, a.H = H, a.W = W;
            a.out_h = t.h, a.out_w = t.w, a.out_wp = t.wp, a.out_hpwp = t.hpwp;
            a.flip = flip;
            e = launch_stem7(dtype, a, s);
            break;
        }
        case OP_MAXPOOL: {
            const Tensor &ti = tensors[pool_in_t], &to = tensors[pool_out_t];
            PoolArgs a;
            a.in = row0(pool_in_t), a.out = row0(pool_out_t);
            a.c = to.c, a.n = nb, a.in_wp = ti.wp, a.in_hpwp = ti.hpwp;
            a.out_h = to.h, a.out_w = to.w, a.out_wp = to.wp, a.out_hpwp = to.hpwp;
            e = launch_maxpool(dtype, a, s);
            break;
        }
        case OP_CONV: {
            const ConvOp &cv = convs[op.idx];
            const ConvArgs a = conv_args(cv, nb, rev);
            e = launch_conv(dtype, a, cv.nr, s);
            break;
        }
        case OP_CONV3_GROUP: {
            Conv3Group &g = groups[op.idx];
            bool hit;
            MapSlot *sl = find_slot(g.slot, nb, &hit);
            if ((e = slot_ready(sl, hit, s)) != hipSuccess) break;
            if (!hit) {
                sl->nblocks = group_blocks(g, nb, &g.map_host, rev);
                if (sl->nblocks > g.map_capacity) {
                    e = hipErrorInvalidValue;
                    break;
                }
                memcpy(sl->pin, g.map_host.data(), (size_t)sl->nblocks * sizeof(int2));
                e = hipMemcpyAsync(sl->dev, sl->pin, (size_t)sl->nblocks * sizeof(int2), hipMemcpyHostToDevice, s);
                if (e == hipSuccess) e = hipEventRecord(sl->landed, s);
                if (e != hipSuccess) break;
                sl->nb = nb;
                ++map_builds;
            }
            e = (dtype == HRN_F16 ? launch_conv3x3_lds_f16 : launch_conv3x3_lds)(probs_dev + g.prob_first, sl->dev, sl->nblocks, nb,
                                                                             convs[g.conv_idx[0]].ks, convs[g.conv_idx[0]].nr, s);
            break;
        }
        case OP_CONV_GROUP: {
            DirectGroup &g = dgroups[op.idx];
            bool hit;
            MapSlot *sl = find_slot(g.slot, nb, &hit);
            if ((e = slot_ready(sl, hit, s)) != hipSuccess) break;
            if (!hit) {
                for (size_t k = 0; k < g.conv_idx.size(); ++k) sl->args_pin[k] = conv_args(convs[g.conv_idx[k]], nb, rev);
                sl->mr = 4;
                while (sl->mr > 1 && direct_group_blocks(g, nb, nullptr, sl->mr) < 512) sl->mr >>= 1;
                sl->nblocks = direct_group_blocks(g, nb, &g.map_host, sl->mr);
                if (sl->nblocks > g.map_capacity) {
                    e = hipErrorInvalidValue;
                    break;
                }
                memcpy(sl->pin, g.map_host.data(), (size_t)sl->nblocks * sizeof(int2));
                e = hipMemcpyAsync(sl->args_dev, sl->args_pin, g.conv_idx.size() * sizeof(ConvArgs), hipMemcpyHostToDevice, s);
                if (e == hipSuccess)
                    e = hipMemcpyAsync(sl->dev, sl->pin, (size_t)sl->nblocks * sizeof(int2), hipMemcpyHostToDevice, s);
                if (e == hipSuccess) e = hipEventRecord(sl->landed, s);
                if (e != hipSuccess) break;
                sl->nb = nb;
                ++map_builds;
            }
            {
                int wl = direct_wlds && is16() ? 1 : 0;
                if (wl)
                    for (int ci : g.conv_idx)
                        if (conv_xl(convs[ci])) wl = 2;
                e = launch_conv_group(dtype, sl->args_dev, sl->dev, sl->nblocks, g.nr, sl->mr, wl, s);
            }
            break;
        }
        case OP_S2_GROUP: {
            S2Group &g = s2groups[op.idx];
            if (!s2_active(g, nb)) {
                for (const Op &f : g.fallback) {
                    e = exec_op(f, rev, images, nb, boxes, box_dtype, pts, heatmaps, s, flip, refine);
                    if (e != hipSuccess) break;
                }
                break;
            }
            bool hit;
            MapSlot *sl = find_slot(g.slot, nb, &hit);
            if ((e = slot_ready(sl, hit, s)) != hipSuccess) break;
            if (!hit) {
                sl->nblocks = s2_blocks(g, nb, &g.map_host);
                if (sl->nblocks > g.map_capacity) {
                    e = hipErrorInvalidValue;
                    break;
                }
                memcpy(sl->pin, g.map_host.data(), (size_t)sl->nblocks * sizeof(int2));
                e = hipMemcpyAsync(sl->dev, sl->pin, (size_t)sl->nblocks * sizeof(int2), hipMemcpyHostToDevice, s);
                if (e == hipSuccess) e = hipEventRecord(sl->landed, s);
                if (e != hipSuccess) break;
                sl->nb = nb;
                ++map_builds;
            }
            e = (dtype == HRN_F16 ? launch_conv_s2_f16 : launch_conv_s2)(s2probs_dev + g.prob_first, sl->dev, sl->nblocks, s);
            break;
        }
        case OP_CHAIN: {
            const Chain &ch = chains[op.idx];
            const ConvOp &c3 = convs[ch.conv3];
            const Tensor &to = tensors[c3.out_t];
            ChainArgs a;
            a.in = row0(c3.in_t), a.res = row0(c3.res_t), a.out_y = row0(c3.out_t);
            a.w3 = blob + c3.w_off, a.b3 = (const float *)(blob + c3.b_off);
            a.out_t = nullptr, a.w1 = nullptr, a.b1 = nullptr;
            if (ch.conv1 >= 0) {
                const ConvOp &c1 = convs[ch.conv1];
                a.out_t = row0(c1.out_t), a.w1 = blob + c1.w_off, a.b1 = (const float *)(blob + c1.b_off);
            }
            a.in3 = nullptr, a.w2 = nullptr, a.b2 = nullptr;
            if (ch.conv2 >= 0) {
                const ConvOp &c2 = convs[ch.conv2];
                a.in3 = row0(c2.in_t), a.w2 = blob + c2.w_off, a.b2 = (const float *)(blob + c2.b_off);
                a.in = nullptr;
            }
            a.x = nullptr, a.wds = nullptr, a.bds = nullptr;
            if (ch.ds >= 0) {
                const ConvOp &cd = convs[ch.ds];
                a.x = row0(cd.in_t), a.wds = blob + cd.w_off, a.bds = (const float *)(blob + cd.b_off);
                a.res = nullptr;
            }
            a.m = nb * to.hpwp, a.h = to.h, a.w = to.w, a.wp = to.wp, a.hpwp = to.hpwp, a.rev = rev, a.max_blocks = chain_blocks;
            e = dtype == HRN_F16 ? launch_bottleneck_chain_f16(a, s) : launch_bottleneck_chain(a, s);
            break;
        }
        case OP_FUSE: {
            FuseGroupArgs ga;
            ga.nf = fuses[op.idx].group;
            for (int k = 0; k < ga.nf; ++k) {
                const FuseOp &f = fuses[op.idx + k];
                const Tensor &to = tensors[f.out_t];
                FuseArgs &a = ga.f[k];
                a.nterms = f.nterms;
                for (int i = 0; i < f.nterms; ++i) {
                    const Tensor &tt = tensors[f.term_t[i]];
                    a.t[i].ptr = row0(f.term_t[i]), a.t[i].shift = f.shift[i];
                    a.t[i].wp = tt.wp, a.t[i].hpwp = tt.hpwp;
                }
                for (int i = f.nterms; i < 4; ++i) a.t[i] = FuseTerm{nullptr, 0, 0, 0};
                a.out = row0(f.out_t), a.c = to.c, a.h = to.h, a.w = to.w, a.wp = to.wp, a.hpwp = to.hpwp;
                a.m = nb * to.hpwp, a.rev = rev;
            }
            e = ga.nf == 1 ? launch_fuse(dtype, ga.f[0], s) : launch_fuse_group(dtype, ga, s);
            break;
        }
        case OP_HEAD: {
            const Tensor &t = tensors[head_in_t];
            HeadArgs a;
            a.in = row0(head_in_t);
            a.wgt = (const float *)(blob + head_w_off), a.bias = (const float *)(blob + head_b_off);
            a.wimg = (is16() && !disable_head_mfma) ? (const void *)(blob + head_wp_off) : nullptr;
            a.heatmaps = heatmaps, a.part_val = part_val, a.part_idx = part_idx;
            a.n = nb, a.c = t.c, a.joints = joints, a.h = t.h, a.w = t.w, a.wp = t.wp, a.hpwp = t.hpwp;
            a.slabs = head_slabs_for(nb), a.slab_px = head_px_for(nb);
            e = launch_head(dtype, a, s);
            break;
        }
        case OP_DECODE: {
            if (!pts) break;
            const Tensor &t = tensors[head_in_t];
            DecodeArgs a{};
            a.part_val = part_val, a.part_idx = part_idx, a.heatmaps = heatmaps, a.boxes = boxes;
            a.box_is_float = box_dtype == HRN_BOX_F32, a.pts = pts;
            a.n = nb, a.joints = joints, a.h = t.h, a.w = t.w, a.slabs = head_slabs_for(nb), a.mode = refine;
            e = launch_decode(a, s);
            break;
        }
    }
        return e;
    }

    bool check_forward_args(const void *images, int n, const void *boxes, float *pts, float *heatmaps, bool outputs_optional = false) {
        if (refuse_plan_only()) return false;
        if (!weights_loaded) {
            err = "weights not loaded (call hrn_load_weights or hrn_adopt_weights)";
            return false;
        }
        if (n < 0 || (n > 0 && !images)) {
            err = "bad images / n";
            return false;
        }
        if (!pts && !heatmaps && !outputs_optional) {
            err = "both pts and heatmaps are NULL";
            return false;
        }
        if (pts && !boxes && n > 0) {
            err = "pts requested without boxes";
            return false;
        }
        return true;
    }
```

### simple-hrnet_amd/csrc/ctx_types.h

```cpp
#pragma once

using namespace hrn;

std::string g_create_error;

struct Tensor {
    int c = 0, h = 0, w = 0;
    int wp = 0, hp = 0, hpwp = 0;
    int buf = -1;
};

struct Buffer {
    int c, h, w;
    size_t lead_rows, rows, bytes;
    char *dev = nullptr;
    bool in_use = false;
};

enum OpKind { OP_STEM, OP_STEM7, OP_MAXPOOL, OP_CONV, OP_CONV3_GROUP, OP_CONV_GROUP, OP_S2_GROUP, OP_CHAIN, OP_FUSE, OP_HEAD, OP_DECODE };

struct ConvOp {
    std::string conv, bn;
    int in_t, out_t, res_t;
    int cin, cout, k, stride, relu;
    int kpad, kchunks, nr;
    int algo = 0;
    int up = 0;
    int ks = 0, slices = 0, ntiles = 0, nch = 0;
    bool n96 = false;
    int fuse_with = -1;
    bool fused_away = false;
    int64_t w_off = 0, w_bytes = 0, b_off = 0;
    bool compact = false;
    bool s2 = false;
    bool w2_image = false;
    int64_t w2_off = 0, w2_bytes = 0;
    double flops = 0;
};

constexpr int kMapSlots = 4;
struct MapSlot {
    int nb = -1;
    int nblocks = 0;
    int mr = 4;
    int2 *dev = nullptr, *pin = nullptr;
    ConvArgs *args_dev = nullptr, *args_pin = nullptr;
    hipEvent_t landed = nullptr;
    hipStream_t up_stream = nullptr;
    uint64_t stamp = 0;
};

struct Conv3Group {
    std::vector<int> conv_idx;
    std::vector<int> fused_prob;
    int prob_first = 0;
    int max_wp = 0;
    int64_t map_capacity = 0;
    MapSlot slot[kMapSlots];
    std::vector<int2> map_host;
};

struct DirectGroup {
    std::vector<int> conv_idx;
    int nr = 0;
    int64_t map_capacity = 0;
    MapSlot slot[kMapSlots];
    std::vector<int2> map_host;
};

struct Op {
    OpKind kind;
    int idx;
};

struct S2Group {
    struct Prob {
        int in_t;
        std::vector<std::pair<int, int>> parts;
        int rows = 1, tiles_per_image = 1;
    };
    std::vector<int> conv_idx;
    std::vector<Prob> probs;
    std::vector<Op> fallback;
    int prob_first = 0;
    int64_t map_capacity = 0;
    MapSlot slot[kMapSlots];
    std::vector<int2> map_host;
};

struct FuseOp {
    int term_t[4];
    int shift[4];
    int nterms;
    int out_t;
    std::string name;
    int group = 1;
};

struct TapPoint {
    std::string name;
    int tensor;
    int op;
    int conv;
};
struct TapReq {
    int op, tensor, crop0, ncrops, crop_step;
    float *dst;
};

inline void fast_div(int d, unsigned *magic, int *shift) {
    int l = 0;
    while ((1 << l) < d) ++l;
    *shift = 30 + l;
    *magic = (unsigned)((1ull << *shift) / (unsigned)d + 1);
}

inline int64_t align_up(int64_t x, int64_t a) { return (x + a - 1) / a * a; }

inline uint16_t f32_to_bf16_host(float f) {
    uint32_t u;
    memcpy(&u, &f, 4);
    u += 0x7fffu + ((u >> 16) & 1u);
    return (uint16_t)(u >> 16);
}

inline uint16_t f32_to_f16_host(float f) {
    uint32_t x;
    memcpy(&x, &f, 4);
    const uint16_t sign = (uint16_t)((x >> 16) & 0x8000u);
    const uint32_t ax = x & 0x7fffffffu;
    if (ax > 0x7f800000u) return sign | 0x7e00u;
    if (ax >= 0x477ff000u) return sign | 0x7c00u;
    if (ax >= 0x38800000u) {
        uint32_t m = ax - 0x38000000u;
        m += 0xfffu + ((m >> 13) & 1u);
        return sign | (uint16_t)(m >> 13);
    }
    float a;
    memcpy(&a, &ax, 4);
    return sign | (uint16_t)std::nearbyint(a * 16777216.0f);
}
```

### simple-hrnet_amd/csrc/hrnet_mi355.cpp

```cpp
#include "../../include/hrnet_mi355.h"

#include <hip/hip_runtime.h>
#include <sys/mman.h>

#include <algorithm>
#include <cmath>
#include <cstdio>
#include <cstdlib>
#include <cstring>
#include <map>
#include <memory>
#include <string>
#include <vector>

#include "assoc_math.h"
#include "letterbox_math.h"
#include "pose_nms_math.h"
#include "kernels.h"
#include "rotate_math.h"
#include "track_geometry.h"

namespace {
#include "ctx_types.h"
}

namespace {
thread_local std::string g_env_seen;
const char *env_sw(const char *name) {
    const char *v = hrn_env(name);
    if (v) {
        const std::string item = std::string(name) + "=" + v + ";";
        if (g_env_seen.find(item) == std::string::npos) g_env_seen += item;
    }
    return v;
}
}

struct hrn_ctx {
    std::string switches;
    int c, joints, H, W, dtype, max_batch, device;
    int model = 0;
    int head_c = 0;
    int pool_in_t = -1, pool_out_t = -1;
    bool plan_only;
    int esize;
    std::string err;
    bool is16() const { return dtype == HRN_BF16 || dtype == HRN_F16; }

    std::vector<Tensor> tensors;
    std::vector<Buffer> buffers;
    std::vector<ConvOp> convs;
    std::vector<FuseOp> fuses;
    std::vector<Conv3Group> groups;
    std::vector<DirectGroup> dgroups;
    std::vector<S2Group> s2groups;
    S2Problem *s2probs_dev = nullptr;
    struct Chain {
        int conv3, conv1, ds;
        int conv2 = -1;
    };
    std::vector<Chain> chains;
    std::vector<TapPoint> taps;
    Conv3Problem *probs_dev = nullptr;
    std::vector<Op> ops;
    int stem_out_t = -1, head_in_t = -1;
    int64_t stem_w_off = 0, stem_b_off = 0, stem_wp_off = 0, head_w_off = 0, head_b_off = 0, head_wp_off = 0;

    int64_t blob_bytes = 0;
    char *blob = nullptr;
    bool weights_loaded = false;

    bool disable_lds = env_sw("HRN_DISABLE_LDS") != nullptr;
    bool assoc_no_assign = env_sw("HRN_ASSOC_NO_ASSIGN") != nullptr;
    bool disable_group = env_sw("HRN_DISABLE_GROUP") != nullptr;
    bool disable_dgroup = env_sw("HRN_DISABLE_DGROUP") != nullptr;
    bool disable_chain = env_sw("HRN_DISABLE_CHAIN") != nullptr;
    bool small_tiles = env_sw("HRN_SMALL_TILES") ? atoi(env_sw("HRN_SMALL_TILES")) != 0 : true;
    int small_below = env_sw("HRN_SMALL_BELOW") ? atoi(env_sw("HRN_SMALL_BELOW")) : 384;
    int small_keep_above = env_sw("HRN_SMALL_KEEP") ? atoi(env_sw("HRN_SMALL_KEEP")) : 300;
    bool disable_chain_ds = env_sw("HRN_DISABLE_CHAIN_DS") != nullptr;
    int pre_mode = env_sw("HRN_PRE_MODE") ? atoi(env_sw("HRN_PRE_MODE")) : 1;
    int chain_blocks = env_sw("HRN_CHAIN_BLOCKS") ? atoi(env_sw("HRN_CHAIN_BLOCKS")) : 512;
    bool disable_chain3 = env_sw("HRN_DISABLE_CHAIN3") != nullptr;
    bool direct_wlds = !(env_sw("HRN_DIRECT_WLDS") && atoi(env_sw("HRN_DIRECT_WLDS")) == 0);
    bool direct_xlds = !(env_sw("HRN_DIRECT_XLDS") && atoi(env_sw("HRN_DIRECT_XLDS")) == 0);
    bool conv_xl(const ConvOp &cv) const {
        return direct_xlds && direct_wlds && is16() && cv.k == 3 && cv.stride == 2 && cv.cin % 32 == 0 && !cv.up && cv.res_t < 0 && cv.nr == 6 &&
               cv.kchunks >= 4;
    }
    bool disable_bbf = env_sw("HRN_BBF") && atoi(env_sw("HRN_BBF")) == 0;
    int bbf_tpb_div = env_sw("HRN_BBF_TPB_DIV") ? std::max(1, atoi(env_sw("HRN_BBF_TPB_DIV"))) : 3;
    double bbf_slide_cost = env_sw("HRN_BBF_SLIDE_COST") ? atof(env_sw("HRN_BBF_SLIDE_COST")) : 24600.0;
    int bbf_min_tiles = env_sw("HRN_BBF_MIN_TILES") ? atoi(env_sw("HRN_BBF_MIN_TILES")) : 1100;
    int dgroup_nr_mode = env_sw("HRN_DGROUP_NR") ? atoi(env_sw("HRN_DGROUP_NR")) : 1;
    bool disable_lds32 = env_sw("HRN_DISABLE_LDS32") != nullptr;
    bool disable_n96 = env_sw("HRN_DISABLE_N96") != nullptr;
    bool disable_fgroup = env_sw("HRN_DISABLE_FGROUP") != nullptr;
    bool disable_f32lds = env_sw("HRN_DISABLE_F32LDS") != nullptr;
    int f32_small_slices = env_sw("HRN_F32_SMALL_SLICES") ? atoi(env_sw("HRN_F32_SMALL_SLICES")) : 0;
    std::vector<Conv3Problem> probs_host;
    bool disable_compact = env_sw("HRN_DISABLE_COMPACT") != nullptr;
    double compact_min_pad = env_sw("HRN_COMPACT_MIN_PAD") ? atof(env_sw("HRN_COMPACT_MIN_PAD")) : 0.08;
    bool disable_s2 = env_sw("HRN_DISABLE_S2") != nullptr;
    int s2_min_tiles = env_sw("HRN_S2_MIN_TILES") ? atoi(env_sw("HRN_S2_MIN_TILES")) : 256;
    int s2_target_blocks = env_sw("HRN_S2_BLOCKS") ? std::max(1, atoi(env_sw("HRN_S2_BLOCKS"))) : 256;
    bool disable_stem_mfma = env_sw("HRN_DISABLE_STEM_MFMA") != nullptr;
    bool disable_stem_fuse = env_sw("HRN_DISABLE_STEM_FUSE") != nullptr;
    bool stem_fuse = false;
    int stem_conv2_op = -1;
    S2Group stemf;
    bool disable_head_mfma = env_sw("HRN_DISABLE_HEAD_MFMA") != nullptr;
    bool direct_nr6 = env_sw("HRN_DIRECT_NR6") ? atoi(env_sw("HRN_DIRECT_NR6")) != 0 : true;
    int half_stages_per_block = env_sw("HRN_HALF_STAGES") ? atoi(env_sw("HRN_HALF_STAGES")) : 8;
    bool alternate = env_sw("HRN_ALTERNATE") ? atoi(env_sw("HRN_ALTERNATE")) != 0 : true;
    int block_order = env_sw("HRN_BLOCK_ORDER") ? atoi(env_sw("HRN_BLOCK_ORDER")) : 1;
    int long_factor = env_sw("HRN_LONG_FACTOR") ? atoi(env_sw("HRN_LONG_FACTOR")) : 4;
    double long_share = env_sw("HRN_LONG_SHARE") ? atof(env_sw("HRN_LONG_SHARE")) : 0.85;
    int head_slabs = 1, head_slab_px = 1024;
    static constexpr int kHeadSlabPxSmall = 256;
    int head_slabs_small = 1;
    int head_px_for(int nb) const { return (long)nb * head_slabs >= 192 ? head_slab_px : kHeadSlabPxSmall; }
    int head_slabs_for(int nb) const { return (long)nb * head_slabs >= 192 ? head_slabs : head_slabs_small; }
    float *part_val = nullptr;
    int *part_idx = nullptr;
    uint64_t map_clock = 0;
    int64_t map_builds = 0;
    float *scratch_hm = nullptr;
    float *scratch_heatmaps() {
        if (!scratch_hm && !hip_ok(hipMalloc((void **)&scratch_hm, (size_t)max_batch * joints * (H / 4) * (W / 4) * sizeof(float)),
                                   "hipMalloc(scratch heat-maps)"))
            scratch_hm = nullptr;
        return scratch_hm;
    }
    int64_t workspace_bytes = 0;

#include "ctx_plan.inc"
#include "ctx_memory.inc"
#include "ctx_weights.inc"
#include "ctx_run.inc"
#include "ctx_scratch.inc"
};

namespace {
using CallScope = hrn_ctx::CallScope;

template <class Pass>
int each_micro_batch(hrn_ctx *h, int n, bool scratch, hipStream_t s, const Pass &pass) {
    if (!h->hip_ok(hipSetDevice(h->device), "hipSetDevice")) return 6;
    if (n == 0) return 0;
    if (scratch && !h->scratch_heatmaps()) return 6;
    CallScope scope(h, &h->pass, s);
    if (!scope.entered) return 6;
    for (int off = 0; off < n; off += h->max_batch)
        if (!pass(off, std::min(n - off, h->max_batch))) return 8;
    return scope.leave() ? 0 : 6;
}

bool valid_refine(hrn_ctx *h, int refine) {
    if (refine == HRN_REFINE_NONE || refine == HRN_REFINE_QUARTER || refine == HRN_REFINE_DARK) return true;
    h->err = "refine must be HRN_REFINE_NONE, HRN_REFINE_QUARTER or HRN_REFINE_DARK";
    return false;
}

const char *bgr_frame_fault(const hrn_frame &f) { return !f.data || f.height <= 0 || f.width <= 0 ? "is null or has no size" : nullptr; }

template <class Frame>
bool frame_table_fault(hrn_handle h, const char *entry, int variant, int n, int nframes, int det_stride, bool pointers, const int32_t *fidx,
                       const Frame *frames, const char *(*frame_fault)(const Frame &)) {
    const std::string name = entry;
    std::string why;
    if (variant != HRN_CROP_PAD && variant != HRN_CROP_CLAMP) why = "variant must be HRN_CROP_PAD or HRN_CROP_CLAMP";
    else if (n < 0 || nframes < 0 || det_stride < 4 || (n > 0 && (nframes < 1 || !pointers))) why = "bad frames / detections / n";
    else if (n > 0 && !fidx && nframes != 1) why = name + ": without frame_index there must be one frame";
    for (int i = 0; why.empty() && i < n; ++i) {
        const long f = fidx ? (long)fidx[i] : 0;
        if (f < 0 || f >= nframes)
            why = name + ": frame_index " + std::to_string(f) + " of person " + std::to_string(i) + " is outside [0, " + std::to_string(nframes) + ")";
        else if (const char *fault = frame_fault(frames[f]))
            why = name + ": frame " + std::to_string(f) + ", which person " + std::to_string(i) + " is cut from, " + fault;
    }
    if (why.empty()) return h->refuse_plan_only();
    h->err = why;
    return true;
}

int forward(hrn_ctx *h, const void *images, int n, const void *boxes, int box_dtype, int refine, float *pts, float *heatmaps,
            hipStream_t s) {
    if (!h) return 1;
    if (!valid_refine(h, refine)) return 7;
    if (!h->check_forward_args(images, n, boxes, pts, heatmaps)) return 7;
    if (refine != HRN_REFINE_NONE && !pts) {
        h->err = "hrn_forward_refined: a refine mode needs pts (it refines the joint coordinates)";
        return 7;
    }
    const bool scratch = refine != HRN_REFINE_NONE && !heatmaps;
    return each_micro_batch(h, n, scratch, s, [&](int off, int nb) {
        const float *img = (const float *)images + (size_t)off * 3 * h->H * h->W;
        const void *bx = boxes ? (const char *)boxes + (size_t)off * 16 : nullptr;
        float *p = pts ? pts + (size_t)off * h->joints * 3 : nullptr;
        float *hp = heatmaps ? heatmaps + (size_t)off * h->joints * (h->H / 4) * (h->W / 4) : scratch ? h->scratch_hm : nullptr;
        return h->run_pass(img, nb, bx, box_dtype, p, hp, s, nullptr, 0, nullptr, refine);
    });
}
}

extern "C" {

const char *hrn_version(void) { return "hrnet_mi355 0.1 (gfx950)"; }

int hrn_create(hrn_handle *out, int c, int nof_joints, int height, int width, int dtype, int max_batch,
               int device_id) {
    return hrn_create_model(out, HRN_MODEL_HRNET, c, nof_joints, height, width, dtype, max_batch, device_id);
}

int hrn_create_model(hrn_handle *out, int model, int c, int nof_joints, int height, int width, int dtype, int max_batch,
                     int device_id) {
    if (!out) return 1;
    *out = nullptr;
    if (model != HRN_MODEL_HRNET && model != HRN_MODEL_POSERESNET) {
        g_create_error = "model must be HRN_MODEL_HRNET or HRN_MODEL_POSERESNET";
        return 2;
    }
    if (model == HRN_MODEL_POSERESNET && c != 50 && c != 101 && c != 152) {
        g_create_error = "PoseResNet: c is the ResNet size, 50 / 101 / 152 (the reference's 18 / 34 cannot run: modules.py:50)";
        return 2;
    }
    if (model == HRN_MODEL_HRNET && (c <= 0 || (c % 32 != 0 && c % 48 != 0))) {
        g_create_error = "c must be a positive multiple of 32 or of 48 (HRNet-W32 / W48 / W64 ...): the kernels tile output channels by 32 / 48 / 64";
        return 2;
    }
    if (height <= 0 || width <= 0 || height % 32 || width % 32) {
        g_create_error = "resolution must be a positive multiple of 32 in both dimensions";
        return 2;
    }
    static_assert(HRN_MAX_JOINTS == kMaxJoints, "the header's bound is the kernels' bound");
    if (nof_joints <= 0 || nof_joints > HRN_MAX_JOINTS) {
        g_create_error = "nof_joints must be in [1, HRN_MAX_JOINTS = " + std::to_string(HRN_MAX_JOINTS) + "]";
        return 2;
    }
    if (dtype != HRN_F32 && dtype != HRN_BF16 && dtype != HRN_F16) {
        g_create_error = "dtype must be HRN_F32, HRN_BF16 or HRN_F16";
        return 2;
    }
    if (max_batch <= 0) {
        g_create_error = "max_batch must be positive";
        return 2;
// ... 1143 lines not shown
        return 7;
    }
    if (n == 0) return 0;
    ScoreArgs a{};
    a.t = (int)(3.0 * sigma);
    a.table = h->score_table(a.t, sigma);
    if (!a.table) return 6;
    hipStream_t s = (hipStream_t)stream;
    const size_t bytes = (size_t)count * sizeof(ScoreJoint);
    if (!h->score_joints.reserve(h, bytes, (size_t)std::max<int64_t>(count, 256 * 17) * sizeof(ScoreJoint), "hipMalloc(score records)")) return 6;
    CallScope scope(h, &h->score_joints, s);
    if (!scope.entered || !h->pre_upload(ring, s, {{h->score_joints.ptr, recs, bytes, "hipMemcpyAsync(score records)"}})) return 6;
    a.joints = h->score_joints.as<ScoreJoint>(), a.n = n, a.J = h->joints, a.h = h->H / 4, a.w = h->W / 4;
    if (!h->hip_ok(launch_targets(a, targets_dev, s), "targets launch")) return 8;
    return scope.leave() ? 0 : 6;
}

int hrn_score_heatmaps(hrn_handle h, const float *heatmaps_dev, int n, const float *targets_dev, const double *joints_host,
                       const float *vis_host, const float *joints_weight_host, double sigma, const float *target_weight_host,
                       float pck_thr, int ohkm_topk, const hrn_score_out *out_dev, void *stream) {
    if (!h) return 1;
    if (h->refuse_plan_only()) return 7;
    if (n < 0 || (n > 0 && !heatmaps_dev)) {
        h->err = "hrn_score_heatmaps: bad heatmaps / n";
        return 7;
    }
    if (((uintptr_t)heatmaps_dev | (uintptr_t)targets_dev) & 15) {
        h->err = "hrn_score_heatmaps: heatmaps / targets must be 16-byte aligned (the maps are read with 16-byte loads)";
        return 7;
    }
    const bool maps = targets_dev != nullptr, analytic = joints_host != nullptr;
    if (maps == analytic) {
        h->err = "hrn_score_heatmaps: give either targets (with target_weight) or joints (with visibility), not both and not neither";
        return 7;
    }
    if (maps ? (!target_weight_host || vis_host || joints_weight_host) : (!vis_host || target_weight_host != nullptr)) {
        h->err = maps ? "hrn_score_heatmaps: target maps come with target_weight and without visibility / joints_weight"
                      : "hrn_score_heatmaps: joints come with visibility and without target_weight";
        return 7;
    }
    if (!std::isfinite(pck_thr)) {
        h->err = "hrn_score_heatmaps: pck_thr is not finite";
        return 7;
    }
    if (ohkm_topk > h->joints) {
        h->err = "hrn_score_heatmaps: ohkm_topk " + std::to_string(ohkm_topk) + " exceeds the " + std::to_string(h->joints) + " joints";
        return 7;
    }
    if (!out_dev || !out_dev->loss_mse || !out_dev->loss_ohkm || !out_dev->avg_acc || !out_dev->cnt || !out_dev->acc ||
        (n > 0 && (!out_dev->dists || !out_dev->map_loss || !out_dev->preds || !out_dev->target_preds || !out_dev->maxvals))) {
        h->err = "hrn_score_heatmaps: every field of hrn_score_out must point to device memory (the per-person ones unless n is 0)";
        return 7;
    }
    if (!h->hip_ok(hipSetDevice(h->device), "hipSetDevice")) return 6;
    const int64_t count = (int64_t)n * h->joints;
    unsigned ring = 0;
    ScoreJoint *recs = (ScoreJoint *)h->pre_stage((size_t)std::max<int64_t>(count, 1) * sizeof(ScoreJoint), &ring);
    if (!recs) return 6;
    ScoreArgs a{};
    if (analytic) {
        const std::string bad = target_centers(joints_host, vis_host, joints_weight_host, n, h->joints, h->H, h->W, sigma, nullptr, nullptr,
                                               nullptr, recs);
        if (!bad.empty()) {
            h->err = "hrn_score_heatmaps: " + bad;
            return 7;
        }
        a.t = (int)(3.0 * sigma);
        a.table = h->score_table(a.t, sigma);
        if (!a.table) return 6;
    } else {
        for (int64_t k = 0; k < count; ++k) recs[k] = ScoreJoint{0, 0, target_weight_host[k], 0};
    }
    hipStream_t s = (hipStream_t)stream;
    const size_t bytes = (size_t)count * sizeof(ScoreJoint);
    if (!h->score_joints.reserve(h, bytes, (size_t)std::max<int64_t>(count, 256 * 17) * sizeof(ScoreJoint), "hipMalloc(score records)")) return 6;
    CallScope scope(h, &h->score_joints, s);
    if (!scope.entered || (count > 0 && !h->pre_upload(ring, s, {{h->score_joints.ptr, recs, bytes, "hipMemcpyAsync(score records)"}}))) return 6;
    a.heatmaps = heatmaps_dev, a.targets = targets_dev, a.joints = h->score_joints.as<ScoreJoint>();
    a.n = n, a.J = h->joints, a.h = h->H / 4, a.w = h->W / 4;
    a.map_loss = out_dev->map_loss, a.preds = out_dev->preds, a.target_preds = out_dev->target_preds, a.maxvals = out_dev->maxvals;
    a.loss_mse = out_dev->loss_mse, a.loss_ohkm = out_dev->loss_ohkm, a.avg_acc = out_dev->avg_acc, a.acc = out_dev->acc;
    a.dists = out_dev->dists, a.cnt = out_dev->cnt, a.pck_thr = pck_thr, a.ohkm_topk = ohkm_topk;
    if (!h->hip_ok(launch_score(a, s), "score launch")) return 8;
    return scope.leave() ? 0 : 6;
}

int hrn_tap_count(hrn_handle h) { return h ? (int)h->taps.size() : 0; }

int hrn_get_tap_info(hrn_handle h, int index, hrn_tap_info *out) {
    if (!h || !out || index < 0 || index >= (int)h->taps.size()) return 1;
    const TapPoint &tp = h->taps[index];
    const Tensor &t = h->tensors[tp.tensor];
    memset(out, 0, sizeof *out);
    snprintf(out->name, sizeof out->name, "%s", tp.name.c_str());
    out->c = t.c, out->h = t.h, out->w = t.w, out->conv_index = tp.conv;
    return 0;
}

int hrn_forward_tap(hrn_handle h, const void *images_dev, int n, const char *tap_name, int crop0, int ncrops, int crop_step,
                    float *dst_dev, float *heatmaps_dev, void *stream) {
    if (!h) return 1;
    if (!h->check_forward_args(images_dev, n, nullptr, nullptr, nullptr, true)) return 7;
    if (!tap_name || !dst_dev || n < 1 || n > h->max_batch || crop0 < 0 || ncrops < 1 || crop_step < 1 ||
        (int64_t)crop0 + (int64_t)(ncrops - 1) * crop_step >= n) {
        h->err = "hrn_forward_tap: needs a tap name, a destination, 1 <= n <= max_batch and crops crop0, crop0 + step, ... inside the call";
        return 7;
    }
    const TapPoint *tp = nullptr;
    for (const TapPoint &t : h->taps)
        if (t.name == tap_name) tp = &t;
    if (!tp) {
        h->err = std::string("hrn_forward_tap: no tensor named '") + tap_name + "' is written by this plan";
        return 7;
    }
    if (tp->conv >= 0 && h->fused_now(h->convs[tp->conv], n)) {
        h->err = std::string("hrn_forward_tap: '") + tap_name + "' stays in LDS at this batch size (fused BasicBlock pass); tap the block's conv2";
        return 7;
    }
    if (!h->hip_ok(hipSetDevice(h->device), "hipSetDevice")) return 6;
    const TapReq req{tp->op, tp->tensor, crop0, ncrops, crop_step, dst_dev};
    CallScope scope(h, &h->pass, (hipStream_t)stream);
    if (!scope.entered) return 6;
    if (!h->run_pass((const float *)images_dev, n, nullptr, 0, nullptr, heatmaps_dev, (hipStream_t)stream, nullptr, 0, &req)) return 8;
    return scope.leave() ? 0 : 6;
}

int hrn_conv_count(hrn_handle h) { return h ? (int)h->convs.size() : 0; }

int hrn_get_conv_info(hrn_handle h, int index, hrn_conv_info *out) {
    if (!h || !out || index < 0 || index >= (int)h->convs.size()) return 1;
    const ConvOp &cv = h->convs[index];
    memset(out, 0, sizeof *out);
    snprintf(out->name, sizeof out->name, "%s", cv.conv.c_str());
    out->cin = cv.cin, out->cout = cv.cout, out->ksize = cv.k, out->stride = cv.stride, out->relu = cv.relu;
    out->has_residual = cv.res_t >= 0;
    out->in_h = h->tensors[cv.in_t].h, out->in_w = h->tensors[cv.in_t].w;
    out->out_h = h->tensors[cv.out_t].h, out->out_w = h->tensors[cv.out_t].w;
    out->kpad = cv.kpad, out->nr = cv.nr, out->algo = cv.fuse_with >= 0 || cv.fused_away ? 2 : cv.n96 ? 3 : cv.s2 ? 4 : cv.algo, out->ks = cv.ks;
    out->w_offset = cv.w_off, out->w_bytes = cv.w_bytes, out->b_offset = cv.b_off;
    out->flops = cv.flops;
    return 0;
}

double hrn_flops_per_crop(hrn_handle h) {
    if (!h) return 0;
    double f = 2.0 * 64 * (h->model == 1 ? 147 : 27) * (h->H / 2) * (double)(h->W / 2);
    for (auto &cv : h->convs) f += cv.flops;
    f += 2.0 * h->joints * h->head_c * (h->H / 4) * (double)(h->W / 4);
    return f;
}

int64_t hrn_workspace_bytes(hrn_handle h) { return h ? h->workspace_bytes : 0; }
int64_t hrn_map_rebuilds(hrn_handle h) { return h ? h->map_builds : -1; }
int hrn_launches_per_pass(hrn_handle h) { return h ? (int)h->ops.size() - (h->stem_fuse ? 1 : 0) : 0; }
int hrn_stem_fused(hrn_handle h) { return h && h->stem_fuse ? 1 : 0; }
int hrn_conv_compact(hrn_handle h, int index) { return h && index >= 0 && index < (int)h->convs.size() && h->convs[index].compact ? 1 : 0; }
const char *hrn_switches(hrn_handle h) { return h ? h->switches.c_str() : ""; }

int64_t hrn_debug_pad_violations(hrn_handle h) {
    if (!h || h->plan_only) return -1;
    if (!h->hip_ok(hipSetDevice(h->device), "hipSetDevice")) return -1;
    unsigned long long *cnt = nullptr, host = 0;
    if (!h->hip_ok(hipMalloc((void **)&cnt, sizeof *cnt), "hipMalloc") || !h->hip_ok(hipMemset(cnt, 0, sizeof *cnt), "hipMemset")) return -1;
    bool ok = h->hip_ok(hipDeviceSynchronize(), "hipDeviceSynchronize");
    for (const Buffer &b : h->buffers) {
        if (!ok) break;
        PadCheckArgs a;
        a.buf = b.dev, a.count = cnt, a.rows = (long)b.rows, a.lead_rows = (long)b.lead_rows;
        a.c = b.c, a.h = b.h, a.w = b.w, a.wp = b.w + 1, a.hpwp = (b.h + 1) * (b.w + 1), a.nmax = h->max_batch;
        ok = h->hip_ok(launch_pad_check(h->dtype, a, nullptr), "pad check launch");
    }
    ok = ok && h->hip_ok(hipMemcpy(&host, cnt, sizeof host, hipMemcpyDeviceToHost), "hipMemcpy");
    (void)hipFree(cnt);
    return ok ? (int64_t)host : -1;
}

int hrn_plan_block_map(hrn_handle h, int group, int n, int reverse, int32_t *blocks, int capacity, int32_t *members, int member_capacity) {
    if (!h || n <= 0 || n > h->max_batch) return -1;
    if (group < 0 || group >= (int)h->groups.size()) return -1;
    const Conv3Group &g = h->groups[group];
    std::vector<int2> map;
    std::vector<int> px;
    const int nblocks = h->group_blocks(g, n, &map, reverse != 0, false, &px);
    for (int i = 0; i < nblocks && i < capacity; ++i) {
        const int x = map[i].x, y = map[i].y;
        int32_t *o = blocks + (size_t)i * 6;
        o[0] = x & 0xff, o[1] = (x >> 8) & 0xff, o[2] = x >> 16, o[3] = y & 0x1fffffff, o[4] = px[i],
        o[5] = ((y >> 29) & 1) | (((y >> 30) & 1) << 1);
    }
    int nm = 0;
    for (size_t k = 0; k < g.conv_idx.size(); ++k, ++nm)
        if (nm < member_capacity) members[nm] = g.conv_idx[k];
    for (size_t k = 0; k < g.conv_idx.size(); ++k)
        if (g.fused_prob[k] >= 0) {
            if (g.fused_prob[k] < member_capacity) members[g.fused_prob[k]] = g.conv_idx[k] | (1 << 30);
            ++nm;
        }
    return nblocks;
}

int hrn_plan_direct_map(hrn_handle h, int group, int n, int32_t *blocks, int capacity, int32_t *members, int member_capacity,
                        int32_t *pixels_per_tile) {
    if (!h || n <= 0 || n > h->max_batch) return -1;
    if (group < 0 || group >= (int)h->dgroups.size()) return -1;
    const DirectGroup &g = h->dgroups[group];
    int mr = 4;
    while (mr > 1 && h->direct_group_blocks(g, n, nullptr, mr) < 512) mr >>= 1;
    std::vector<int2> map;
    const int nblocks = h->direct_group_blocks(g, n, &map, mr);
    for (int i = 0; i < nblocks && i < capacity; ++i)
        blocks[(size_t)i * 3] = map[i].x & 0xff, blocks[(size_t)i * 3 + 1] = map[i].x >> 8, blocks[(size_t)i * 3 + 2] = map[i].y;
    for (size_t k = 0; k < g.conv_idx.size() && (int)k < member_capacity; ++k) members[k] = g.conv_idx[k];
    if (pixels_per_tile) *pixels_per_tile = 64 * mr;
    return nblocks;
}

int hrn_plan_s2_map(hrn_handle h, int group, int n, int32_t *blocks, int capacity, int32_t *parts, int part_capacity, int32_t *active) {
    if (!h || n <= 0 || n > h->max_batch) return -1;
    if (group == -1 && !h->stem_fuse) return -1;
    if (group < -1 || group >= (int)h->s2groups.size()) return -1;
    const S2Group &g = group == -1 ? h->stemf : h->s2groups[group];
    std::vector<int2> map;
    const int nblocks = h->s2_blocks(g, n, &map);
    for (int i = 0; i < nblocks && i < capacity; ++i)
        blocks[(size_t)i * 3] = map[i].x & 0xff, blocks[(size_t)i * 3 + 1] = map[i].x >> 8, blocks[(size_t)i * 3 + 2] = map[i].y;
    int np = 0;
    for (size_t k = 0; k < g.probs.size(); ++k)
        for (auto &pt : g.probs[k].parts) {
            if (np < part_capacity) {
                int32_t *o = parts + (size_t)np * 5;
                o[0] = (int32_t)k, o[1] = pt.first, o[2] = pt.second, o[3] = g.probs[k].rows, o[4] = g.probs[k].tiles_per_image;
            }
            ++np;
        }
    if (active) *active = h->s2_active(g, n) ? 1 : 0;
    return nblocks | (np << 20);
}

int hrn_plan_head_slabs(hrn_handle h, int n, int32_t *slab_px) {
    if (!h || n <= 0 || n > h->max_batch) return -1;
    if (slab_px) *slab_px = h->head_px_for(n);
    return h->head_slabs_for(n);
}

int hrn_plan_launch_walk(hrn_handle h, int kind, int index, int n, int32_t *out) {
    if (!h || !out || n <= 0 || n > h->max_batch || index < 0) return -1;
    if (kind != 0 && kind != 1) return -1;
    if (index >= (int)(kind == 0 ? h->groups.size() : h->chains.size())) return -1;
    int pos = -1;
    for (size_t oi = 0; oi < h->ops.size(); ++oi)
        if (h->ops[oi].kind == (kind == 0 ? OP_CONV3_GROUP : OP_CHAIN) && h->ops[oi].idx == index) pos = (int)oi;
    if (pos < 0) return -1;
    out[0] = pos, out[1] = h->alternate && (pos & 1) ? 1 : 0, out[2] = out[3] = out[4] = 0;
    if (kind == 1) {
        const auto &ch = h->chains[index];
        out[4] = ch.conv2 >= 0 ? (ch.conv1 >= 0 ? 2 : 3) : ch.ds >= 0 ? 1 : 0;
        const int m = n * h->tensors[h->convs[ch.conv3].out_t].hpwp;
        out[2] = chain_waves(ch.ds >= 0, ch.conv2 >= 0) * chain_grid(m, ch.ds >= 0, ch.conv2 >= 0, h->chain_blocks);
        out[3] = (m + 15) / 16;
    }
    return 0;
}

int hrn_profile_pass(hrn_handle h, const void *images_dev, int n, float *conv_ms, int conv_ms_len, float *other_ms,
                     void *stream) {
    if (!h) return 1;
    if (n > h->max_batch) n = h->max_batch;
    if (!h->check_forward_args(images_dev, n, nullptr, nullptr, nullptr, true)) return 7;
    if (!h->hip_ok(hipSetDevice(h->device), "hipSetDevice")) return 6;
    hrn_ctx::Timing tm;
    tm.ev.resize(h->ops.size() + 1);
    for (auto &e : tm.ev)
        if (!h->hip_ok(hipEventCreate(&e), "hipEventCreate")) return 6;
    CallScope scope(h, &h->pass, (hipStream_t)stream);
    bool ok = scope.entered && h->run_pass((const float *)images_dev, n, nullptr, 0, nullptr, nullptr, (hipStream_t)stream, &tm) && scope.leave();
    ok = ok && h->hip_ok(hipStreamSynchronize((hipStream_t)stream), "hipStreamSynchronize");
    if (ok) {
        if (other_ms) other_ms[0] = other_ms[1] = other_ms[2] = other_ms[3] = 0.f;
        for (int i = 0; i < conv_ms_len; ++i) conv_ms[i] = 0.f;
        for (size_t oi = 0; oi < h->ops.size(); ++oi) {
            float ms = 0.f;
            (void)hipEventElapsedTime(&ms, tm.ev[oi], tm.ev[oi + 1]);
            const Op &op = h->ops[oi];
            if (op.kind == OP_CONV) {
                if (conv_ms && op.idx < conv_ms_len) conv_ms[op.idx] = ms;
            } else if (op.kind == OP_CONV3_GROUP) {
                const Conv3Group &g = h->groups[op.idx];
                double tot = 0;
                for (int ci : g.conv_idx) {
                    const ConvOp &cv = h->convs[ci];
                    if (h->skipped(cv, n)) continue;
                    tot += cv.flops + (h->fused_now(cv, n) ? h->convs[cv.fuse_with].flops : 0.0);
                }
                for (int ci : g.conv_idx) {
                    const ConvOp &cv = h->convs[ci];
                    if (h->skipped(cv, n)) continue;
                    if (conv_ms && ci < conv_ms_len) conv_ms[ci] = (float)(ms * cv.flops / tot);
                    const int c2 = h->fused_now(cv, n) ? cv.fuse_with : -1;
                    if (conv_ms && c2 >= 0 && c2 < conv_ms_len) conv_ms[c2] = (float)(ms * h->convs[c2].flops / tot);
                }
            } else if (op.kind == OP_CONV_GROUP) {
                const DirectGroup &g = h->dgroups[op.idx];
                double tot = 0;
                std::vector<double> wgt;
                for (int ci : g.conv_idx) {
                    const ConvOp &cv = h->convs[ci];
                    wgt.push_back((double)h->grid_of(cv).hpwp * (cv.cout / (16 * g.nr)) * cv.kchunks);
                    tot += wgt.back();
                }
                for (size_t k = 0; k < g.conv_idx.size(); ++k)
                    if (conv_ms && g.conv_idx[k] < conv_ms_len) conv_ms[g.conv_idx[k]] = (float)(ms * wgt[k] / tot);
            } else if (op.kind == OP_S2_GROUP) {
                const S2Group &g = h->s2groups[op.idx];
                double tot = 0;
                for (int ci : g.conv_idx) tot += h->convs[ci].flops;
                for (int ci : g.conv_idx)
                    if (conv_ms && ci < conv_ms_len) conv_ms[ci] = (float)(ms * h->convs[ci].flops / tot);
            } else if (op.kind == OP_CHAIN) {
                const hrn_ctx::Chain &ch = h->chains[op.idx];
                double tot = 0;
                for (int ci : {ch.conv3, ch.conv1, ch.ds, ch.conv2})
                    if (ci >= 0) tot += h->convs[ci].flops;
                for (int ci : {ch.conv3, ch.conv1, ch.ds, ch.conv2})
                    if (conv_ms && ci >= 0 && ci < conv_ms_len) conv_ms[ci] = (float)(ms * h->convs[ci].flops / tot);
            } else if (other_ms) {
                const int slot = (op.kind == OP_STEM || op.kind == OP_STEM7 || op.kind == OP_MAXPOOL) ? 0 : op.kind == OP_FUSE ? 1 : op.kind == OP_HEAD ? 2 : 3;
                other_ms[slot] += ms;
            }
        }
    }
    for (auto &e : tm.ev) (void)hipEventDestroy(e);
    return ok ? 0 : 8;
}

}
```

### simple-hrnet_amd/csrc/kernels.h

```cpp
#pragma once
#include <hip/hip_runtime.h>
#include <stdint.h>

#include <atomic>
#include <cstdlib>
#include <cstring>

namespace hrn {

inline hipError_t set_dynamic_lds(const void *func, int bytes, std::atomic<unsigned long long> &done) {
    int dev = 0;
    hipError_t e = hipGetDevice(&dev);
    if (e != hipSuccess) return e;
    const unsigned long long bit = 1ull << (dev & 63);
    if (done.load(std::memory_order_acquire) & bit) return hipSuccess;
    e = hipFuncSetAttribute(func, hipFuncAttributeMaxDynamicSharedMemorySize, bytes);
    if (e == hipSuccess) done.fetch_or(bit, std::memory_order_release);
    return e;
}

inline const char *hrn_env(const char *name) {
    static const bool debug = [] {
        const char *v = getenv("HRN_DEBUG_ENV");
        return v && *v && strcmp(v, "0") != 0;
    }();
    return debug ? getenv(name) : nullptr;
}

enum { DT_F32 = 0, DT_BF16 = 1, DT_F16 = 2 };

struct ConvArgs {
    const void *in;
    void *out;
    const void *w;
    const float *bias;
    const void *res;
    int cin, cout;
    int in_wp, in_hpwp;
    int out_h, out_w, out_wp, out_hpwp;
    int m;
    int ksize, stride, relu;
    int kchunks;
    int rev;
    int pre_mode;
    int wlds;
    int xlds;
    int up, up_a, up_b, up_wp, up_hpwp;
    int taps[4];
};

struct Conv3Problem {
    const void *in;
    void *out;
    const void *w;
    const float *bias;
    const void *res;
    int cin, cout;
    int h, wd, wp, hpwp;
    int relu;
    int slices;
    int ntiles;
    int tiles_per_block;
    int bm;
    unsigned magic_hpwp, magic_wp;
    int shift_hpwp, shift_wp;
    const void *w2;
    const float *bias2;
    int n96;
    int compact, hw;
    unsigned magic_hw, magic_w;
    int shift_hw, shift_w;
    int slab_rows, slab_rows_small;
};
int conv3x3_n96_ch64();
int conv3x3_lds_bbf_ok(int wp);
int conv3x3_n96_max_rows();
int conv3x3_lds_bm(int ks, int nrb, int wp);
int conv3x3_f32_bm(int wp);
hipError_t launch_conv3x3_f32(const Conv3Problem *probs_dev, const void *blockmap_dev, int nblocks, int nb, int nrb, hipStream_t s);

constexpr int kS2SlabBytes = 79872;
constexpr int s2_frags_per_part(int cin) { return cin == 48 ? 3 : 2; }
constexpr int s2_subslot_bytes(int cin) { return cin % 48 == 0 ? 96 : 32; }
constexpr int s2_region_bytes(int cin) { return kS2SlabBytes / (cin * 2 / s2_subslot_bytes(cin)) / 1024 * 1024; }
constexpr int s2_slot_capacity(int cin) { return s2_region_bytes(cin) / s2_subslot_bytes(cin); }
constexpr int s2_pair_pad(int wop) { return (8 - (3 * wop) % 8) % 8; }
constexpr int s2_pair_pitch(int wop) { return 4 * wop + s2_pair_pad(wop); }
constexpr int kS2MaxParts = 8;
struct S2Part {
    const void *w;
    const float *bias;
    void *out;
    int cout, ch0;
    int relu, pad_;
};
struct S2Problem {
    const void *in;
    int cin;
    int in_wp, in_hpwp;
    int ho, wo, wop, out_hpwp;
    int rows;
    int tiles_per_image;
    int nparts;
    unsigned char wave_part[8], wave_f0[8], wave_fs[8];
    unsigned magic_wop;
    int shift_wop;
    S2Part part[kS2MaxParts];
};
hipError_t launch_conv_s2(const S2Problem *probs_dev, const void *map_dev, int nblocks, hipStream_t s);
hipError_t launch_conv_s2_f16(const S2Problem *probs_dev, const void *map_dev, int nblocks, hipStream_t s);

constexpr int kStemFuseRegionBytes = 15360;
constexpr int kStemFusePatchBytes = 12544;
int stem_fused_fits(int wop, int w_in);

struct ChainArgs {
    const void *in;
    const void *res;
    void *out_y;
    void *out_t;
    const void *w3;
    const float *b3;
    const void *w1;
    const float *b1;
    const void *in3;
    const void *w2;
    const float *b2;
    const void *x;
    const void *wds;
    const float *bds;
    int m, h, w, wp, hpwp;
    int rev;
    int max_blocks;
};
constexpr int chain_waves(bool ds, bool c3) { return c3 || ds ? 8 : 4; }
inline int chain_grid(int m, bool ds, bool c3, int max_blocks) {
    const int blocks_env = max_blocks > 0 ? max_blocks : 512;
    const int waves = chain_waves(ds, c3), mfrags = (m + 15) / 16;
    const int blocks = (mfrags + waves - 1) / waves;
    const int cap = (ds || c3) ? (blocks_env / 2 > 1 ? blocks_env / 2 : 1) : blocks_env;
    return blocks > cap ? cap : blocks;
}
hipError_t launch_bottleneck_chain(const ChainArgs &a, hipStream_t s);
hipError_t launch_bottleneck_chain_f16(const ChainArgs &a, hipStream_t s);

struct StemArgs {
    const float *images;
    void *out;
    const float *w;
    const float *bias;
    const void *wp;
    int n, H, W;
    int out_h, out_w, out_wp, out_hpwp;
    int flip;
};

hipError_t launch_stem_fused(int dtype, const S2Problem *probs_dev, const void *map_dev, int nblocks, const StemArgs &stem, hipStream_t s);

struct CropParams {
    int x1, y1, w_crop, h_crop;
    int pad_top, pad_left;
    int h_pad, w_pad;
    long long tmp_off;
    const unsigned char *frame;
    int frame_w, frame_h;
};
hipError_t launch_prepath(const CropParams *crops_dev, int n, int max_h_pad, unsigned char *tmp_dev, float *images_dev, int H, int W,
                          hipStream_t s);
struct YuvSource {
    const unsigned char *y, *u, *v;
    int pitch_y, pitch_c;
    int format;
    int coef[6];
    int pad_;
};
hipError_t launch_prepath_yuv(const CropParams *crops_dev, const YuvSource *src_dev, int n, int max_h_pad, unsigned char *tmp_dev,
                              float *images_dev, int H, int W, hipStream_t s);
hipError_t launch_yuv_to_bgr(const YuvSource &src, int height, int width, unsigned char *bgr_dev, hipStream_t s);
struct ResizeTaps {
    int ofs;
    short c[4];
};
inline double resize_scale(int dst, int src) { return 1.0 / ((double)dst / (double)src); }
hipError_t launch_resize_frames(const unsigned char *frames_dev, int n, int src_h, int src_w, int interp, ResizeTaps *taps_dev,
                                float *images_dev, int H, int W, hipStream_t s);
struct WarpParams {
    double m[6];
    int frame;
    int pad_;
};
hipError_t launch_warp_crops(const unsigned char *frames_dev, int frame_h, int frame_w, const WarpParams *params_dev, int n,
                             float *images_dev, int H, int W, hipStream_t s);

struct Stem7Args {
    const float *images;
    void *out;
    const float *w;
    const float *bias;
    const void *wp;
    int n, H, W;
    int out_h, out_w, out_wp, out_hpwp;
    int flip;
};
struct PoolArgs {
    const void *in;
    void *out;
    int c, n;
    int in_wp, in_hpwp;
    int out_h, out_w, out_wp, out_hpwp;
};
hipError_t launch_stem7(int dtype, const Stem7Args &a, hipStream_t s);
hipError_t launch_maxpool(int dtype, const PoolArgs &a, hipStream_t s);

struct FuseTerm {
    const void *ptr;
    int shift;
    int wp, hpwp;
};
struct FuseArgs {
    FuseTerm t[4];
    int nterms;
    void *out;
    int c, h, w, wp, hpwp;
    int m;
    int rev;
// ... 248 lines not shown
```

Measured before the change: 11620 crops/s.

## Absorb stage fuse-0 sum into last branch-0 basic-block fused conv epilogue

Defers the final branch-0 basic-block fused conv of multi-branch stages until after the cross-resolution terms are computed. Its epilogue then adds the upsampled low-resolution addends, loaded with nearest-neighbour indexing and prefetched during the last K chunk, and applies ReLU before writing the fuse output directly. This is meant to remove the separate fuse pass over the large high-resolution tensor and one intermediate write and read. In exchange it adds planner complexity (deferred groups, op position bookkeeping, tap handling, map keys), extra registers in the kernel epilogue, and a later dependency point for the conv.

Result: no change. 11630 crops/s, median of 3 (+0.1%).

```diff
diff --git a/include/hrnet_mi355.h b/include/hrnet_mi355.h
--- a/include/hrnet_mi355.h
+++ b/include/hrnet_mi355.h
@@ -246,6 +246,7 @@
                     int32_t *active);
 int hrn_plan_head_slabs(hrn_handle h, int n, int32_t *slab_px);
 int hrn_plan_launch_walk(hrn_handle h, int kind, int index, int n, int32_t *out);
+int hrn_plan_ops(hrn_handle h, int32_t *out, int capacity);
 int hrn_profile_pass(hrn_handle h, const void *images_dev, int n, float *conv_ms, int conv_ms_len,
                      float *other_ms , void *stream);
 const char *hrn_version(void);
diff --git a/simple-hrnet_amd/_lib.py b/simple-hrnet_amd/_lib.py
--- a/simple-hrnet_amd/_lib.py
+++ b/simple-hrnet_amd/_lib.py
@@ -275,6 +275,7 @@
     "hrn_plan_s2_map": (ctypes.c_int, [_P, ctypes.c_int, ctypes.c_int, _P, ctypes.c_int, _P, ctypes.c_int, _P]),
     "hrn_plan_head_slabs": (ctypes.c_int, [_P, ctypes.c_int, _P]),
     "hrn_plan_launch_walk": (ctypes.c_int, [_P, ctypes.c_int, ctypes.c_int, ctypes.c_int, _P]),
+    "hrn_plan_ops": (ctypes.c_int, [_P, _P, ctypes.c_int]),
     "hrn_profile_pass": (ctypes.c_int, [_P, _P, ctypes.c_int, ctypes.POINTER(ctypes.c_float), ctypes.c_int,
                                         ctypes.POINTER(ctypes.c_float), _P]),
     "hrn_version": (ctypes.c_char_p, []),
diff --git a/simple-hrnet_amd/csrc/conv3x3_lds.inc b/simple-hrnet_amd/csrc/conv3x3_lds.inc
--- a/simple-hrnet_amd/csrc/conv3x3_lds.inc
+++ b/simple-hrnet_amd/csrc/conv3x3_lds.inc
@@ -475,7 +475,7 @@
     __builtin_amdgcn_s_barrier();
 }
 
-template <int DT>
+template <int DT, int NZ>
 __device__ __forceinline__ void bbf_run(const Conv3Problem &p, const int mt0, const int tiles_this_block, const int nb, char *smem) {
     constexpr int KS = 48, NRB = 3, ROWB = 96, NCH = 14, BM = 512, MR = 4, NT = 512;
     typedef __attribute__((ext_vector_type(2))) unsigned u32x2;
@@ -556,9 +556,11 @@
         for (int k = NXR; k < NXP; ++k)
             if (xu0 + k * NT + wave * 64 < xunits) glds16((const GLOBAL_AS char *)x_src(tt, k), xy + (xu0 + k * NT + wave * 64) * 16);
     };
+    constexpr bool ADD = NZ > 0;
+    constexpr int ZA = 2;
     auto store_x = [&]() {
         const unsigned a0 = lds0 + 2 * BBF_W + (xu0 + tid) * 16;
-        asm volatile("s_waitcnt vmcnt(0)" ::: "memory");
+        asm volatile("s_waitcnt vmcnt(%0)" ::"i"(2 * NZ * MR) : "memory");
 #pragma unroll
         for (int k = 0; k < NXR; ++k)
             asm volatile("ds_write_b128 %0, %1 offset:%2" ::"v"(a0), "v"(xpre[k]), "i"(k * NT * 16) : "memory");
@@ -617,6 +619,28 @@
             okbits2 |= ((q < m) && (ho < p.h) && (wo < p.wd)) ? 1u << i : 0u;
         }
         __builtin_amdgcn_sched_barrier(0);
+        u32x4 zq[MR][ADD ? NZ : 1];
+        u32x2 zd[MR][ADD ? NZ : 1];
+        auto issue_z = [&](const int i0, const int i1) {
+#pragma unroll
+            for (int i = 0; i < MR; ++i) {
+                if (i < i0 || i >= i1) continue;
+                int q = (int)p0 + wave * 16 * MR + i * 16 + li;
+                asm volatile("" : "+v"(q));
+                const int n_img = (int)(((unsigned long long)(unsigned)q * p.magic_hpwp) >> p.shift_hpwp);
+                const int rem = q - n_img * p.hpwp;
+                const int ho = (int)(((unsigned long long)(unsigned)rem * p.magic_wp) >> p.shift_wp);
+                const int wo = rem - ho * p.wp;
+#pragma unroll
+                for (int k = 0; k < NZ; ++k) {
+                    const unsigned row = q < m ? (unsigned)(n_img * p.z[k].hpwp + (ho >> (k + 1)) * p.z[k].wp + (wo >> (k + 1))) : 0u;
+                    const unsigned zo = row * (KS * 2) + ch0 * 2;
+                    asm volatile("s_nop 4\n\tglobal_load_dwordx4 %0, %2, %3\n\tglobal_load_dwordx2 %1, %2, %3 offset:16"
+                                 : "=&v"(zq[i][k]), "=&v"(zd[i][k])
+                                 : "v"(zo), "s"(p.z[k].ptr));
+                }
+            }
+        };
         f32x4 acc[MR][NRB];
         {
             float bias2[4 * NRB];
@@ -646,6 +670,9 @@
                 const int cur = c & 1, nxt = cur ^ 1;
                 if (c + 1 < NCH) {
                     BBF_READ2(nxt, c + 1)
+                }
+                if (ADD && c == NCH - 1) issue_z(0, ZA);
+                if (c + 1 < NCH) {
                     asm volatile("s_waitcnt lgkmcnt(%0)" ::"i"(NRB + MR) : "memory");
                 } else {
                     asm volatile("s_waitcnt lgkmcnt(0)" ::: "memory");
@@ -665,6 +692,7 @@
 #undef BBF_READ2
         }
         C3_T(tE);
+        if (ADD) issue_z(ZA, MR);
         asm volatile("s_waitcnt lgkmcnt(0)" ::: "memory");
         __builtin_amdgcn_s_barrier();
         if (carry) {
@@ -673,6 +701,10 @@
         }
         __builtin_amdgcn_sched_barrier(0);
         C3_T(tF);
+        if (ADD) {
+            asm volatile("s_waitcnt vmcnt(0)" ::: "memory");
+            __builtin_amdgcn_sched_barrier(0);
+        }
 #pragma unroll
         for (int i = 0; i < MR; ++i) {
             const int q = (int)p0 + wave * 16 * MR + i * 16 + li;
@@ -687,7 +719,16 @@
                 float v2 = acc[i][j][2] + H16<DT>::lo(r23);
                 float v3 = acc[i][j][3] + H16<DT>::hi(r23);
                 if (p.relu) v0 = relu1(v0), v1 = relu1(v1), v2 = relu1(v2), v3 = relu1(v3);
-                const unsigned lo = H16<DT>::pk(v0, v1), hi = H16<DT>::pk(v2, v3);
+                unsigned lo = H16<DT>::pk(v0, v1), hi = H16<DT>::pk(v2, v3);
+                if (ADD) {
+                    float s0 = H16<DT>::lo(lo), s1 = H16<DT>::hi(lo), s2 = H16<DT>::lo(hi), s3 = H16<DT>::hi(hi);
+#pragma unroll
+                    for (int k = 0; k < NZ; ++k) {
+                        const unsigned z01 = j < 2 ? zq[i][k][2 * j] : zd[i][k][0], z23 = j < 2 ? zq[i][k][2 * j + 1] : zd[i][k][1];
+                        s0 += H16<DT>::lo(z01), s1 += H16<DT>::hi(z01), s2 += H16<DT>::lo(z23), s3 += H16<DT>::hi(z23);
+                    }
+                    lo = H16<DT>::pk(relu1(s0), relu1(s1)), hi = H16<DT>::pk(relu1(s2), relu1(s3));
+                }
                 pk[2 * j] = ok ? lo : 0u;
                 pk[2 * j + 1] = ok ? hi : 0u;
             }
@@ -738,7 +779,14 @@
     const int mt0 = bm.y & 0x1fffffff;
     if constexpr (KS == 48 && NRB == 3) {
         if (bm.y & (1 << 29)) {
-            bbf_run<DT>(p, mt0, tiles, nb, smem);
+            if (p.nz == 0)
+                bbf_run<DT, 0>(p, mt0, tiles, nb, smem);
+            else if (p.nz == 1)
+                bbf_run<DT, 1>(p, mt0, tiles, nb, smem);
+            else if (p.nz == 2)
+                bbf_run<DT, 2>(p, mt0, tiles, nb, smem);
+            else
+                bbf_run<DT, 3>(p, mt0, tiles, nb, smem);
             return;
         }
         if (p.n96) {
diff --git a/simple-hrnet_amd/csrc/ctx_memory.inc b/simple-hrnet_amd/csrc/ctx_memory.inc
--- a/simple-hrnet_amd/csrc/ctx_memory.inc
+++ b/simple-hrnet_amd/csrc/ctx_memory.inc
@@ -45,6 +45,28 @@
     }
     bool fused_now(const ConvOp &cv, int nb) const { return cv.fuse_with >= 0 && bbf_active(cv, nb); }
     bool skipped(const ConvOp &cv, int nb) const { return cv.fused_away && bbf_active(cv, nb); }
+    bool absorbs(const ConvOp &cv, int nb) const {
+        return cv.defer_group >= 0 && fused_now(cv, nb) && cur_tap_tensor != convs[cv.fuse_with].out_t;
+    }
+    bool group_skips(const Conv3Group &g, const ConvOp &cv, int nb) const {
+        return g.deferred ? !absorbs(cv, nb) : skipped(cv, nb) || absorbs(cv, nb);
+    }
+    int group_index(int number) const {
+        int k = number < 0 ? -1 - number : number;
+        for (size_t i = 0; i < groups.size(); ++i)
+            if (groups[i].deferred == (number < 0) && k-- == 0) return (int)i;
+        return -1;
+    }
+    int group_number(int index) const {
+        int k = 0;
+        for (int i = 0; i < index; ++i) k += groups[i].deferred == groups[index].deferred ? 1 : 0;
+        return groups[index].deferred ? -1 - k : k;
+    }
+    int map_key(const Conv3Group &g, int nb) const {
+        for (int ci : g.conv_idx)
+            if (absorbs(convs[ci], nb)) return nb | (1 << 30);
+        return nb;
+    }
 
     int group_blocks(const Conv3Group &g, int nb, std::vector<int2> *out, bool reverse, bool all_short = false,
                      std::vector<int> *tile_px_out = nullptr) const {
@@ -57,7 +79,7 @@
         long one_per_block = 0;
         for (int ci : g.conv_idx) {
             const ConvOp &cv = convs[ci];
-            if (skipped(cv, nb)) continue;
+            if (group_skips(g, cv, nb)) continue;
             const Tensor &to = tensors[cv.out_t];
             const int bmn = fused_now(cv, nb) ? 512 : conv3x3_lds_bm(cv.ks, cv.nr, to.wp);
             one_per_block += (long)((m_pixels(cv, to, nb) + bmn - 1) / bmn) * cv.ntiles;
@@ -66,7 +88,7 @@
         long small_blocks = 0;
         for (int ci : g.conv_idx) {
             const ConvOp &cv = convs[ci];
-            if (skipped(cv, nb)) continue;
+            if (group_skips(g, cv, nb)) continue;
             small_blocks += (long)((m_pixels(cv, tensors[cv.out_t], nb) + 127) / 128) * cv.ntiles;
         }
         const bool keep_short_full = small && small_keep_above > 0 && small_blocks > small_keep_above;
@@ -85,7 +107,7 @@
             long total = 0;
             for (int ci : g.conv_idx) {
                 const ConvOp &cv = convs[ci];
-                if (skipped(cv, nb)) continue;
+                if (group_skips(g, cv, nb)) continue;
                 const Tensor &to = tensors[cv.out_t];
                 const int bm = tile_px(cv, to);
                 const int mtiles = (int)((m_pixels(cv, to, nb) + bm - 1) / bm);
@@ -100,7 +122,7 @@
         if (lf < 1) lf = 1;
         for (size_t k = 0; k < g.conv_idx.size(); ++k) {
             const ConvOp &cv = convs[g.conv_idx[k]];
-            if (skipped(cv, nb)) continue;
+            if (group_skips(g, cv, nb)) continue;
             const Tensor &to = tensors[cv.out_t];
             const int bm = tile_px(cv, to);
             const bool fused = fused_now(cv, nb);
@@ -437,6 +459,12 @@
                     f = q;
                     f.out = row0(c2.out_t), f.relu = c2.relu, f.res = nullptr;
                     f.w2 = blob + c2.w_off, f.bias2 = (const float *)(blob + c2.b_off);
+                    if (g.deferred) {
+                        const FuseOp &fo = fuses[g.fuse0];
+                        f.out = row0(fo.out_t), f.nz = fo.nterms - 1;
+                        for (int j = 1; j < fo.nterms; ++j)
+                            f.z[j - 1] = Conv3Addend{row0(fo.term_t[j]), tensors[fo.term_t[j]].wp, tensors[fo.term_t[j]].hpwp};
+                    }
                 }
             }
         }
diff --git a/simple-hrnet_amd/csrc/ctx_plan.inc b/simple-hrnet_amd/csrc/ctx_plan.inc
--- a/simple-hrnet_amd/csrc/ctx_plan.inc
+++ b/simple-hrnet_amd/csrc/ctx_plan.inc
@@ -118,6 +118,8 @@
         }
     }
 
+    int deferred_conv = -1;
+
     void emit_convs(const std::vector<int> &idx) {
         std::vector<int> lds, direct, s2;
         for (int i : idx) {
@@ -129,6 +131,14 @@
                 direct.push_back(i);
         }
         emit_direct(direct, ops);
+        if (deferred_conv >= 0 && !direct.empty()) {
+            Conv3Group g;
+            g.conv_idx = {deferred_conv}, g.deferred = true;
+            groups.push_back(g);
+            convs[deferred_conv].defer_group = (int)groups.size() - 1;
+            ops.push_back({OP_CONV3_GROUP, (int)groups.size() - 1});
+            deferred_conv = -1;
+        }
         if (!s2.empty()) {
             S2Group g;
             g.conv_idx = s2;
@@ -193,6 +203,7 @@
     void add_stage(const std::string &name, std::vector<int> &xs, int nout) {
         const int nb = (int)xs.size();
         char buf[160];
+        int absorb_conv = -1, absorb_x = -1;
         for (int k = 0; k < 4; ++k) {
             std::vector<int> t1(nb), g1, g2;
             for (int b = 0; b < nb; ++b) {
@@ -212,6 +223,7 @@
                     a1.ntiles == 1 && a2.slices == 1 && a2.ntiles == 1 && conv3x3_lds_bbf_ok(tensors[t2].wp)) {
                     convs[i1].fuse_with = i2;
                     convs[i2].fused_away = true;
+                    if (k == 3 && b == 0 && nb > 1 && nout == 1 && !disable_fuse0) absorb_conv = i1, absorb_x = xs[b];
                 }
                 g2.push_back(i2);
                 release(t1[b]);
@@ -222,6 +234,7 @@
         }
         std::vector<std::vector<int>> term(nout, std::vector<int>(nb, -1));
         std::vector<std::vector<int>> cur(nout, std::vector<int>(nb, -1));
+        deferred_conv = absorb_conv;
         for (int level = 0; level < nb; ++level) {
             std::vector<int> made, dead;
             for (int j = 0; j < nb; ++j) {
@@ -256,6 +269,7 @@
             emit_convs(made);
             for (int t : dead) release(t);
         }
+        deferred_conv = -1;
         std::vector<int> outs;
         for (int i = 0; i < nout; ++i) {
             std::vector<int> terms, shifts;
@@ -264,7 +278,14 @@
                 shifts.push_back(i < j ? j - i : 0);
             }
             snprintf(buf, sizeof buf, "%s.fuse.%d", name.c_str(), i);
+            const bool absorbed = i == 0 && absorb_conv >= 0 && convs[absorb_conv].defer_group >= 0;
+            if (absorbed) buffers[tensors[absorb_x].buf].in_use = true;
             outs.push_back(add_fuse(terms, shifts, buf));
+            if (absorbed) {
+                buffers[tensors[absorb_x].buf].in_use = false;
+                fuses.back().absorb_conv = absorb_conv;
+                groups[convs[absorb_conv].defer_group].fuse0 = (int)fuses.size() - 1;
+            }
         }
         {
             const int first = (int)fuses.size() - nout;
@@ -443,8 +464,12 @@
                 }
             taps.push_back(TapPoint{name, tensor, op, conv});
         };
+        int pos = 0;
         for (size_t oi = 0; oi < ops.size(); ++oi) {
-            const Op &op = ops[oi];
+            Op &op = ops[oi];
+            const bool deferred = op.kind == OP_CONV3_GROUP && groups[op.idx].deferred;
+            op.pos = deferred ? pos : pos++;
+            if (deferred) continue;
             switch (op.kind) {
                 case OP_STEM:
                 case OP_STEM7: add("stem", stem_out_t, (int)oi, -1); break;
diff --git a/simple-hrnet_amd/csrc/ctx_run.inc b/simple-hrnet_amd/csrc/ctx_run.inc
--- a/simple-hrnet_amd/csrc/ctx_run.inc
+++ b/simple-hrnet_amd/csrc/ctx_run.inc
@@ -5,9 +5,14 @@
     bool run_pass(const float *images, int nb, const void *boxes, int box_dtype, float *pts, float *heatmaps,
                   hipStream_t s, Timing *tm, int flip = 0, const TapReq *tap = nullptr, int refine = RF_NONE) {
         if (tm && !hip_ok(hipEventRecord(tm->ev[0], s), "hipEventRecord")) return false;
+        struct TapScope {
+            int &t;
+            ~TapScope() { t = -1; }
+        } tap_scope{cur_tap_tensor};
+        cur_tap_tensor = tap ? tap->tensor : -1;
         const bool fused_stem = stem_fuse && !(tap && tap->op == 0);
         for (size_t oi = 0; oi < ops.size(); ++oi) {
-            const bool rev = alternate && (oi & 1);
+            const bool rev = alternate && (ops[oi].pos & 1);
             hipError_t e = hipSuccess;
             if (fused_stem && oi == 0)
                 e = exec_stem_fused(images, nb, s, flip);
@@ -98,8 +103,10 @@
         }
         case OP_CONV3_GROUP: {
             Conv3Group &g = groups[op.idx];
+            if (g.deferred && !absorbs(convs[g.conv_idx[0]], nb)) break;
             bool hit;
-            MapSlot *sl = find_slot(g.slot, nb, &hit);
+            const int key = map_key(g, nb);
+            MapSlot *sl = find_slot(g.slot, key, &hit);
             if ((e = slot_ready(sl, hit, s)) != hipSuccess) break;
             if (!hit) {
                 sl->nblocks = group_blocks(g, nb, &g.map_host, rev);
@@ -111,7 +118,7 @@
                 e = hipMemcpyAsync(sl->dev, sl->pin, (size_t)sl->nblocks * sizeof(int2), hipMemcpyHostToDevice, s);
                 if (e == hipSuccess) e = hipEventRecord(sl->landed, s);
                 if (e != hipSuccess) break;
-                sl->nb = nb;
+                sl->nb = key;
                 ++map_builds;
             }
             e = (dtype == HRN_F16 ? launch_conv3x3_lds_f16 : launch_conv3x3_lds)(probs_dev + g.prob_first, sl->dev, sl->nblocks, nb,
@@ -208,9 +215,11 @@
         }
         case OP_FUSE: {
             FuseGroupArgs ga;
-            ga.nf = fuses[op.idx].group;
+            const int k0 = fuses[op.idx].absorb_conv >= 0 && absorbs(convs[fuses[op.idx].absorb_conv], nb) ? 1 : 0;
+            ga.nf = fuses[op.idx].group - k0;
+            if (ga.nf <= 0) break;
             for (int k = 0; k < ga.nf; ++k) {
-                const FuseOp &f = fuses[op.idx + k];
+                const FuseOp &f = fuses[op.idx + k0 + k];
                 const Tensor &to = tensors[f.out_t];
                 FuseArgs &a = ga.f[k];
                 a.nterms = f.nterms;
diff --git a/simple-hrnet_amd/csrc/ctx_types.h b/simple-hrnet_amd/csrc/ctx_types.h
--- a/simple-hrnet_amd/csrc/ctx_types.h
+++ b/simple-hrnet_amd/csrc/ctx_types.h
@@ -30,6 +30,7 @@
     bool n96 = false;
     int fuse_with = -1;
     bool fused_away = false;
+    int defer_group = -1;
     int64_t w_off = 0, w_bytes = 0, b_off = 0;
     bool compact = false;
     bool s2 = false;
@@ -53,6 +54,8 @@
 struct Conv3Group {
     std::vector<int> conv_idx;
     std::vector<int> fused_prob;
+    bool deferred = false;
+    int fuse0 = -1;
     int prob_first = 0;
     int max_wp = 0;
     int64_t map_capacity = 0;
@@ -71,6 +74,7 @@
 struct Op {
     OpKind kind;
     int idx;
+    int pos = 0;
 };
 
 struct S2Group {
@@ -95,6 +99,7 @@
     int out_t;
     std::string name;
     int group = 1;
+    int absorb_conv = -1;
 };
 
 struct TapPoint {
diff --git a/simple-hrnet_amd/csrc/hrnet_mi355.cpp b/simple-hrnet_amd/csrc/hrnet_mi355.cpp
--- a/simple-hrnet_amd/csrc/hrnet_mi355.cpp
+++ b/simple-hrnet_amd/csrc/hrnet_mi355.cpp
@@ -92,6 +92,8 @@
     int bbf_tpb_div = env_sw("HRN_BBF_TPB_DIV") ? std::max(1, atoi(env_sw("HRN_BBF_TPB_DIV"))) : 3;
     double bbf_slide_cost = env_sw("HRN_BBF_SLIDE_COST") ? atof(env_sw("HRN_BBF_SLIDE_COST")) : 24600.0;
     int bbf_min_tiles = env_sw("HRN_BBF_MIN_TILES") ? atoi(env_sw("HRN_BBF_MIN_TILES")) : 1100;
+    bool disable_fuse0 = env_sw("HRN_FUSE0_ABSORB") && atoi(env_sw("HRN_FUSE0_ABSORB")) == 0;
+    int cur_tap_tensor = -1;
     int dgroup_nr_mode = env_sw("HRN_DGROUP_NR") ? atoi(env_sw("HRN_DGROUP_NR")) : 1;
     bool disable_lds32 = env_sw("HRN_DISABLE_LDS32") != nullptr;
     bool disable_n96 = env_sw("HRN_DISABLE_N96") != nullptr;
@@ -1541,7 +1543,12 @@
 
 int64_t hrn_workspace_bytes(hrn_handle h) { return h ? h->workspace_bytes : 0; }
 int64_t hrn_map_rebuilds(hrn_handle h) { return h ? h->map_builds : -1; }
-int hrn_launches_per_pass(hrn_handle h) { return h ? (int)h->ops.size() - (h->stem_fuse ? 1 : 0) : 0; }
+int hrn_launches_per_pass(hrn_handle h) {
+    if (!h) return 0;
+    int n = (int)h->ops.size() - (h->stem_fuse ? 1 : 0);
+    for (const Conv3Group &g : h->groups) n -= g.deferred ? 1 : 0;
+    return n;
+}
 int hrn_stem_fused(hrn_handle h) { return h && h->stem_fuse ? 1 : 0; }
 int hrn_conv_compact(hrn_handle h, int index) { return h && index >= 0 && index < (int)h->convs.size() && h->convs[index].compact ? 1 : 0; }
 const char *hrn_switches(hrn_handle h) { return h ? h->switches.c_str() : ""; }
@@ -1566,11 +1573,23 @@
 
 int hrn_plan_block_map(hrn_handle h, int group, int n, int reverse, int32_t *blocks, int capacity, int32_t *members, int member_capacity) {
     if (!h || n <= 0 || n > h->max_batch) return -1;
-    if (group < 0 || group >= (int)h->groups.size()) return -1;
-    const Conv3Group &g = h->groups[group];
+    if (h->group_index(group) < 0) return -1;
+    const Conv3Group &g = h->groups[h->group_index(group)];
     std::vector<int2> map;
     std::vector<int> px;
-    const int nblocks = h->group_blocks(g, n, &map, reverse != 0, false, &px);
+    int nblocks = h->group_blocks(g, n, &map, reverse != 0, false, &px);
+    for (size_t k = 0; k < g.conv_idx.size() && !g.deferred; ++k) {
+        const ConvOp &cv = h->convs[g.conv_idx[k]];
+        if (!h->absorbs(cv, n)) continue;
+        std::vector<int2> dmap;
+        std::vector<int> dpx;
+        const int nd = h->group_blocks(h->groups[cv.defer_group], n, &dmap, reverse != 0, false, &dpx);
+        for (int i = 0; i < nd; ++i) {
+            map.push_back(int2{(dmap[i].x & ~0xff) | g.fused_prob[k], dmap[i].y});
+            px.push_back(dpx[i]);
+        }
+        nblocks += nd;
+    }
     for (int i = 0; i < nblocks && i < capacity; ++i) {
         const int x = map[i].x, y = map[i].y;
         int32_t *o = blocks + (size_t)i * 6;
@@ -1633,14 +1652,15 @@
 }
 
 int hrn_plan_launch_walk(hrn_handle h, int kind, int index, int n, int32_t *out) {
-    if (!h || !out || n <= 0 || n > h->max_batch || index < 0) return -1;
+    if (!h || !out || n <= 0 || n > h->max_batch || (index < 0 && kind != 0)) return -1;
     if (kind != 0 && kind != 1) return -1;
-    if (index >= (int)(kind == 0 ? h->groups.size() : h->chains.size())) return -1;
+    if (kind == 0) index = h->group_index(index);
+    if (index < 0 || index >= (int)(kind == 0 ? h->groups.size() : h->chains.size())) return -1;
     int pos = -1;
     for (size_t oi = 0; oi < h->ops.size(); ++oi)
         if (h->ops[oi].kind == (kind == 0 ? OP_CONV3_GROUP : OP_CHAIN) && h->ops[oi].idx == index) pos = (int)oi;
     if (pos < 0) return -1;
-    out[0] = pos, out[1] = h->alternate && (pos & 1) ? 1 : 0, out[2] = out[3] = out[4] = 0;
+    out[0] = pos, out[1] = h->alternate && (h->ops[pos].pos & 1) ? 1 : 0, out[2] = out[3] = out[4] = 0;
     if (kind == 1) {
         const auto &ch = h->chains[index];
         out[4] = ch.conv2 >= 0 ? (ch.conv1 >= 0 ? 2 : 3) : ch.ds >= 0 ? 1 : 0;
@@ -1649,6 +1669,16 @@
         out[3] = (m + 15) / 16;
     }
     return 0;
+}
+
+int hrn_plan_ops(hrn_handle h, int32_t *out, int capacity) {
+    if (!h) return -1;
+    for (size_t oi = 0; oi < h->ops.size() && (int)oi < capacity && out; ++oi) {
+        const Op &op = h->ops[oi];
+        out[4 * oi] = (int32_t)op.kind, out[4 * oi + 1] = op.kind == OP_CONV3_GROUP ? h->group_number(op.idx) : op.idx, out[4 * oi + 2] = op.pos;
+        out[4 * oi + 3] = op.kind == OP_CONV3_GROUP && h->groups[op.idx].deferred ? 1 : 0;
+    }
+    return (int)h->ops.size();
 }
 
 int hrn_profile_pass(hrn_handle h, const void *images_dev, int n, float *conv_ms, int conv_ms_len, float *other_ms,
@@ -1678,12 +1708,12 @@
                 double tot = 0;
                 for (int ci : g.conv_idx) {
                     const ConvOp &cv = h->convs[ci];
-                    if (h->skipped(cv, n)) continue;
+                    if (h->group_skips(g, cv, n)) continue;
                     tot += cv.flops + (h->fused_now(cv, n) ? h->convs[cv.fuse_with].flops : 0.0);
                 }
                 for (int ci : g.conv_idx) {
                     const ConvOp &cv = h->convs[ci];
-                    if (h->skipped(cv, n)) continue;
+                    if (h->group_skips(g, cv, n)) continue;
                     if (conv_ms && ci < conv_ms_len) conv_ms[ci] = (float)(ms * cv.flops / tot);
                     const int c2 = h->fused_now(cv, n) ? cv.fuse_with : -1;
                     if (conv_ms && c2 >= 0 && c2 < conv_ms_len) conv_ms[c2] = (float)(ms * h->convs[c2].flops / tot);
diff --git a/simple-hrnet_amd/csrc/kernels.h b/simple-hrnet_amd/csrc/kernels.h
--- a/simple-hrnet_amd/csrc/kernels.h
+++ b/simple-hrnet_amd/csrc/kernels.h
@@ -49,6 +49,10 @@
     int taps[4];
 };
 
+struct Conv3Addend {
+    const void *ptr;
+    int wp, hpwp;
+};
 struct Conv3Problem {
     const void *in;
     void *out;
@@ -71,6 +75,8 @@
     unsigned magic_hw, magic_w;
     int shift_hw, shift_w;
     int slab_rows, slab_rows_small;
+    int nz;
+    Conv3Addend z[3];
 };
 int conv3x3_n96_ch64();
 int conv3x3_lds_bbf_ok(int wp);
```
